# lightalchemist/nonlocal-image-edit

Hardware: AMD Instinct MI355X
Metric: megapixels/sec end-to-end enhance (4K img, m=200, K=50); device-resident input and output (host->host per SURVEY 8d: host_to_host.value) (higher is better)
Workload: dtype f64; 1 GPU; cfg4: 4096x4096 synthetic luminance, 20x10 samples (p=200), K=50, T=10, L=4 layers; device-resident: the luminance plane is in HBM when the timed region starts and the 4 layer planes are left in HBM (no PCIe inside `value`); parallelism=single GPU, formulation=phi_free_tables, storage=fp64 tables, histograms, reductions and MFMA; fp32 output planes

## Files before the change

include/nle.h:

```cpp
#ifndef NLE_H
#define NLE_H

#include <stddef.h>

#ifdef __cplusplus
extern "C" {
#endif

#define NLE_OK 0
#define NLE_ERR_INVALID 1
#define NLE_ERR_HIP 2
#define NLE_ERR_NUMERIC 3
#define NLE_ERR_COMM 4

#define NLE_EPS 1e-10

typedef struct nle_ctx nle_ctx;
typedef struct nle_filter nle_filter;

int nle_ctx_create(int device, void* stream, nle_ctx** out);
void nle_ctx_destroy(nle_ctx* ctx);
const char* nle_last_error(const nle_ctx* ctx);
int nle_ctx_synchronize(nle_ctx* ctx);
int nle_ctx_trim(nle_ctx* ctx);

int nle_dev_alloc(nle_ctx* ctx, size_t bytes, void** d_ptr);
void nle_dev_free(nle_ctx* ctx, void* d_ptr);
int nle_host_alloc(nle_ctx* ctx, size_t bytes, void** h_ptr);
void nle_host_free(nle_ctx* ctx, void* h_ptr);
int nle_dev_upload(nle_ctx* ctx, void* d_dst, const void* h_src, size_t bytes);
int nle_dev_download(nle_ctx* ctx, void* h_dst, const void* d_src, size_t bytes);

#define NLE_MODE_AUTO 0
#define NLE_MODE_MATERIALISED 1
#define NLE_MODE_PHI_FREE 2
#define NLE_MODE_PHI_FREE_EXP 3
#define NLE_MODE_MATERIALISED_F64 4
#define NLE_MODE_STREAMED_F64 5
#define NLE_MODE_EXACT_F64 6
#define NLE_EXACT_MAX_PIXELS 1048576
int nle_ctx_set_mode(nle_ctx* ctx, int mode);
#define NLE_PATCH_RADIUS_MAX 7
int nle_ctx_set_patch_radius(nle_ctx* ctx, int radius);
#define NLE_CHROMA_PATCH_RADIUS_MAX 3
int nle_ctx_set_chroma(nle_ctx* ctx, const float* d_a, const float* d_b, double hc);
int nle_filter_chroma(const nle_filter* f, double* hc);
#define NLE_SAMPLER_GRID 0
#define NLE_SAMPLER_FARTHEST 1
int nle_ctx_set_sampler(nle_ctx* ctx, int sampler);
int nle_sample_pixels(nle_ctx* ctx, const float* d_lum, int H, int W, int n_row_samples, int n_col_samples, double hx,
                      double hy, long long* h_idx, int* p);
int nle_ctx_set_nystrom_bf16x3(nle_ctx* ctx, int on);

int nle_ctx_set_slab_input(nle_ctx* ctx, int on);

int nle_ctx_set_topk_solver(nle_ctx* ctx, int solver);

#define NLE_RCCL_UNIQUE_ID_BYTES 128
int nle_rccl_unique_id(void* h_id, size_t size);
int nle_ctx_init_rccl(nle_ctx* ctx, int rank, int world, const void* h_id, size_t size);
int nle_ctx_set_rccl_comm(nle_ctx* ctx, int rank, int world, void* nccl_comm);
int nle_ctx_abort_rccl(nle_ctx* ctx);
typedef int (*nle_allreduce_fn)(void* user, void* d_buf, size_t count);
int nle_ctx_set_shard(nle_ctx* ctx, int rank, int world, nle_allreduce_fn allreduce,
                      void* user, double* d_comm, size_t comm_len);
size_t nle_comm_len(int n_samples);

int nle_sample_grid(int H, int W, int n_row_samples, int n_col_samples, int* row_step,
                    int* row_off, int* n_sel_rows, int* col_step, int* col_off,
                    int* n_sel_cols);
int nle_slab_rows(int H, int rank, int world, int* row0, int* row1);
int nle_eigen_decomposition(const double* h_M, int n, double eps, double* h_U, double* h_D,
                            int* r);
int nle_eigen_decomposition_top(const double* h_M, int n, double eps, int kmax, double* h_U, double* h_D, int* r);
int nle_eigen_decomposition_topk(const double* h_M, int n, double eps, int kmax, double* h_U, double* h_Dk, int* r);
int nle_eigen_decomposition_top_device(nle_ctx* ctx, const double* h_M, int n, double eps, int kmax, double* h_U, double* h_D,
                                       int* r);
int nle_sym_eigen_device(nle_ctx* ctx, const double* h_M, int n, double eps, int first, int count, double* h_U, double* h_D,
                         int* r);
int nle_cholesky_device(nle_ctx* ctx, const double* h_M, int n, double* h_L, double* h_Linv, double* inv_trace, int* ok);
int nle_topk_eigen_decomposition(const double* h_M, int n, int n_largest, double eps, double* h_U, double* h_D, int* r);
int nle_transform_eigenvalues(const double* h_eigvals, int K, const double* h_weights, int L,
                              double* h_fS);
int nle_layer_responses(const double* h_eigvals, int K, int L, double* h_resp);

int nle_compute_kernel(nle_ctx* ctx, const float* d_lum, int H, int W, int n_row_samples,
                       int n_col_samples, double hx, double hy, double* h_Ka, float* d_kab);
int nle_nystrom(nle_ctx* ctx, const float* d_lum, int H, int W, int n_row_samples,
                int n_col_samples, double hx, double hy, double* h_eigvals, int* r,
                float* d_phi);
int nle_ts_gemm(nle_ctx* ctx, const float* d_A, long long M, int lda, int kd,
                const double* h_B, int nc, float* d_C);
int nle_sinkhorn_scalings(nle_ctx* ctx, const float* d_phi, long long M, int ld, int r,
                          const double* h_eigvals, int max_iter, double* h_u_c,
                          double* h_u_r);
int nle_gram(nle_ctx* ctx, const float* d_phi, long long M, int ld, int r, const double* h_u,
             double* h_G);
int nle_row_scalings(nle_ctx* ctx, const float* d_phi, long long M, int ld, int r,
                     const double* h_u, double* d_out);

int nle_compute_kernel64(nle_ctx* ctx, const float* d_lum, int H, int W, int n_row_samples, int n_col_samples, double hx,
                         double hy, double* h_Ka, double* d_kab);
int nle_ts_gemm64(nle_ctx* ctx, const double* d_A, long long M, int lda, int kd, const double* h_B, int nc, double* d_C);
int nle_sinkhorn_scalings64(nle_ctx* ctx, const double* d_phi, long long M, int ld, int r, const double* h_eigvals,
                            int max_iter, double* h_u_c, double* h_u_r);
int nle_gram64(nle_ctx* ctx, const double* d_phi, long long M, int ld, int r, const double* h_u, double* h_G);
int nle_row_scalings64(nle_ctx* ctx, const double* d_phi, long long M, int ld, int r, const double* h_u, double* d_out);
int nle_affinity_product64(nle_ctx* ctx, const float* d_lum, int H, int W, double hx, double hy, const double* d_X, int ld,
                           int ncols, double* d_Y);

int nle_train(nle_ctx* ctx, const float* d_lum, int H, int W, int n_row_samples,
              int n_col_samples, double hx, double hy, int n_sinkhorn_iter,
              int n_eigen_vectors, nle_filter** out);
int nle_train_host(nle_ctx* ctx, const float* h_lum, int H, int W, int n_row_samples,
                   int n_col_samples, double hx, double hy, int n_sinkhorn_iter,
                   int n_eigen_vectors, nle_filter** out);
int nle_train_host_u8(nle_ctx* ctx, const unsigned char* h_lum8, int H, int W, int n_row_samples,
                      int n_col_samples, double hx, double hy, int n_sinkhorn_iter,
                      int n_eigen_vectors, nle_filter** out);
void nle_filter_destroy(nle_filter* f);
int nle_filter_info(const nle_filter* f, long long* n_local, int* K, int* r, int* p,
                    int* row0, int* row1);
int nle_filter_diag(const nle_filter* f, int* h_info);
int nle_filter_eigvals(const nle_filter* f, double* h_eigvals );
int nle_filter_sample_pixels(const nle_filter* f, long long* h_idx, int* p);
int nle_filter_eigvec_range(const nle_filter* f, int ncols, double* h_min, double* h_max);
int nle_filter_eigvecs(const nle_filter* f, const float** d_V, int* ld);
int nle_filter_copy_eigvecs(const nle_filter* f, float* d_out);
int nle_filter_timings(const nle_filter* f, double* h_ms);

int nle_apply(nle_filter* f, const float* d_x, int H, int W, const double* h_fS, float* d_y);
int nle_apply_layers(nle_filter* f, const float* d_x, int H, int W, int L, float* d_y);
int nle_apply_host(nle_filter* f, const float* h_x, int H, int W, const double* h_fS,
                   float* h_y);
int nle_apply_layers_host(nle_filter* f, const float* h_x, int H, int W, int L, float* h_y);
int nle_apply_u8(nle_filter* f, const float* d_x, int H, int W, const double* h_fS, unsigned char* d_out);
int nle_apply_rounded8(nle_filter* f, const float* d_x, int H, int W, const double* h_fS, float* d_y);
int nle_apply_u8_host(nle_filter* f, const float* h_x, int H, int W, const double* h_fS, unsigned char* h_out);

int nle_bgr2lab8(nle_ctx* ctx, const unsigned char* d_bgr, long long n, unsigned char* d_lab, float* d_L);
int nle_lab8_tables(unsigned short* h_gamma, unsigned short* h_cbrt, int* h_coeffs);
int nle_lab8_inverse_tables(unsigned short* h_yf, int* h_ab_to_xz, unsigned short* h_inv_gamma, int* h_coeffs);
int nle_lab2bgr8(nle_ctx* ctx, const unsigned char* d_lab, const float* d_L, long long n, unsigned char* d_bgr);
int nle_lab2bgr8_planes(nle_ctx* ctx, const unsigned char* d_lab, const float* d_L, const float* d_a, const float* d_b,
                        long long n, unsigned char* d_bgr);
int nle_lab8_channel(nle_ctx* ctx, const unsigned char* d_lab, long long n, int channel, float* d_out);

int nle_bilateral8(nle_ctx* ctx, const float* d_src, int H, int W, double sigma_color, double sigma_space, float* d_dst);
int nle_bilateral_tables(double sigma_color, double sigma_space, int* radius, float* h_space_w, float* h_colour_w);

int nle_ld(int n);

enum {
    NLE_K_AFFINITY = 0,
    NLE_K_NYSTROM = 1,
    NLE_K_SINKHORN_PASS = 2,
    NLE_K_REDUCE = 3,
    NLE_K_GRAM = 4,
    NLE_K_PROJECT = 5,
    NLE_K_APPLY_REDUCE = 6,
    NLE_K_APPLY_EXPAND = 7,
    NLE_K_SMALL = 8,
    NLE_K_SINK_TABLES = 9,
    NLE_K_GRAM_ROWS = 10,
    NLE_K_GRAM_GEMM = 11,
    NLE_KERNEL_COUNT = 12
};
const char* nle_kernel_name(int kid);
int nle_ctx_profile(nle_ctx* ctx, int enable);
int nle_ctx_kernel_stats(nle_ctx* ctx, int kid, long long* launches, double* total_ms);
int nle_bench_affinity(nle_ctx* ctx, const float* d_lum, int H, int W, int n_row_samples,
                       int n_col_samples, double hx, double hy, float* d_kab, int reps,
                       double* h_avg_ms);
int nle_bench_affinity64(nle_ctx* ctx, const float* d_lum, int H, int W, int n_row_samples, int n_col_samples, double hx,
                         double hy, long long rows, double* d_kab, int reps, double* h_avg_ms);
int nle_filter_level_tiles(const nle_filter* f, int* first_tile, int* n_tiles);
int nle_bench_sinkhorn_pass(nle_ctx* ctx, const float* d_phi, long long M, int ld, int r,
                            int reps, double* h_avg_ms);

#ifdef __cplusplus
}
#endif
#endif
```

nonlocal-image-edit_amd/__init__.py:

```python
from __future__ import annotations

import ctypes as C
import os

import numpy as np

_HERE = os.path.dirname(os.path.abspath(__file__))
LIB_PATH = os.path.join(_HERE, "lib", "libnle_hip.so")

from . import _abi
from ._abi import (ALLREDUCE_FN, NLE_ERR_COMM, NLE_ERR_HIP, NLE_ERR_INVALID, NLE_ERR_NUMERIC, NLE_OK)

EPS = 1e-10
KERNEL_COUNT = _abi.NLE_KERNEL_COUNT
_P = C.c_void_p
_SIGNATURES = _abi.SIGNATURES
EXPORTED_SYMBOLS = tuple(_SIGNATURES)
MODE_AUTO, MODE_MATERIALISED, MODE_PHI_FREE, MODE_PHI_FREE_EXP, MODE_MATERIALISED_F64, MODE_STREAMED_F64 = (
    _abi.NLE_MODE_AUTO, _abi.NLE_MODE_MATERIALISED, _abi.NLE_MODE_PHI_FREE, _abi.NLE_MODE_PHI_FREE_EXP,
    _abi.NLE_MODE_MATERIALISED_F64, _abi.NLE_MODE_STREAMED_F64)
MODE_EXACT_F64 = _abi.NLE_MODE_EXACT_F64
EXACT_MAX_PIXELS = _abi.NLE_EXACT_MAX_PIXELS
SAMPLER_GRID, SAMPLER_FARTHEST = _abi.NLE_SAMPLER_GRID, _abi.NLE_SAMPLER_FARTHEST

# ... 390 lines not shown
                                        float(hx), float(hy), _np_ptr(Ka),
                                        C.c_void_p(kab.data_ptr()) if want_kab else None), self._h)
        return np.ascontiguousarray(Ka), kab

    def nystrom(self, lum, n_row_samples, n_col_samples, hx, hy):
        torch = _torch()
        lum = self._lum(lum)
        H, W = lum.shape
        if n_row_samples > H or n_col_samples > W:
            raise NLEError(NLE_ERR_INVALID, "Number of samples per row and col must be <= that of image.")
        g = sample_grid(H, W, n_row_samples, n_col_samples)
        p = g["n_sel_rows"] * g["n_sel_cols"]
        n_local = self.local_pixels(H, W)
        buf = torch.empty(n_local * ld(p), dtype=torch.float32, device=lum.device)
        ev = np.zeros(p, dtype=np.float64)
        r = C.c_int()
        _check(lib().nle_nystrom(self._h, C.c_void_p(lum.data_ptr()), H, W, n_row_samples, n_col_samples, float(hx),
                                 float(hy), _np_ptr(ev), C.byref(r), C.c_void_p(buf.data_ptr())), self._h)
        rr = r.value
        return ev[:rr].copy(), buf[: n_local * ld(rr)].view(n_local, ld(rr)), rr

    def ts_gemm(self, A, kd, B):
        torch = _torch()
        self._sync_in()
        B = np.asfortranarray(np.asarray(B, dtype=np.float64))
        M, lda = A.shape
        nc = B.shape[1]
        Cc = torch.empty((M, ld(nc)), dtype=torch.float32, device=A.device)
        _check(lib().nle_ts_gemm(self._h, C.c_void_p(A.data_ptr()), M, lda, kd, _np_ptr(B), nc,
                                 C.c_void_p(Cc.data_ptr())), self._h)
        return Cc

    def sinkhorn_scalings(self, phi, r, eigvals, max_iter=10):
        ev = np.ascontiguousarray(eigvals, dtype=np.float64)
        uc, ur = np.zeros(r), np.zeros(r)
        self._sync_in()
        M, ldp = phi.shape
        _check(lib().nle_sinkhorn_scalings(self._h, C.c_void_p(phi.data_ptr()), M, ldp, r, _np_ptr(ev), max_iter,
                                           _np_ptr(uc), _np_ptr(ur)), self._h)
        return uc, ur

    def gram(self, phi, r, u):
        self._sync_in()
        u = np.ascontiguousarray(u, dtype=np.float64)
        G = np.zeros((r, r), dtype=np.float64, order="F")
        M, ldp = phi.shape
        _check(lib().nle_gram(self._h, C.c_void_p(phi.data_ptr()), M, ldp, r, _np_ptr(u), _np_ptr(G)), self._h)
        return np.ascontiguousarray(G)

    def row_scalings(self, phi, r, u):
        torch = _torch()
        self._sync_in()
        u = np.ascontiguousarray(u, dtype=np.float64)
        M, ldp = phi.shape
        out = torch.empty(M, dtype=torch.float64, device=phi.device)
        _check(lib().nle_row_scalings(self._h, C.c_void_p(phi.data_ptr()), M, ldp, r, _np_ptr(u),
                                      C.c_void_p(out.data_ptr())), self._h)
        return out

    def _mat64(self, X, width, what):
        torch = _torch()
        if X.dtype != torch.float64 or X.ndim != 2 or not X.is_cuda:
            raise NLEError(NLE_ERR_INVALID, f"{what}: need a float64 device tensor (M, ld)")
        M, ldx = X.shape
        if X.stride(1) != 1 or (M > 1 and X.stride(0) != ldx):
            raise NLEError(NLE_ERR_INVALID, f"{what}: rows must be contiguous with stride ld")
        if not 1 <= width <= ldx:
            raise NLEError(NLE_ERR_INVALID, f"{what}: need 1 <= logical width <= ld")
        self._sync_in()
        return M, ldx

    def ts_gemm64(self, A, kd, B):
        torch = _torch()
        M, lda = self._mat64(A, kd, "ts_gemm64")
        B = np.asfortranarray(np.asarray(B, dtype=np.float64))
        if B.ndim != 2 or B.shape[0] != kd:
            raise NLEError(NLE_ERR_INVALID, "ts_gemm64: B must be kd x nc")
        nc = B.shape[1]
        Cc = torch.empty((M, ld(nc)), dtype=torch.float64, device=A.device)
        _check(lib().nle_ts_gemm64(self._h, C.c_void_p(A.data_ptr()), M, lda, kd, _np_ptr(B), nc,
                                   C.c_void_p(Cc.data_ptr())), self._h)
        return Cc

    def sinkhorn_scalings64(self, phi, r, eigvals, max_iter=10):
        M, ldp = self._mat64(phi, r, "sinkhorn_scalings64")
        ev = np.ascontiguousarray(eigvals, dtype=np.float64)
        if ev.size < r:
            raise NLEError(NLE_ERR_INVALID, "sinkhorn_scalings64: need r eigenvalues")
        uc, ur = np.zeros(r), np.zeros(r)
        _check(lib().nle_sinkhorn_scalings64(self._h, C.c_void_p(phi.data_ptr()), M, ldp, r, _np_ptr(ev), max_iter,
                                             _np_ptr(uc), _np_ptr(ur)), self._h)
        return uc, ur

    def gram64(self, phi, r, u=None):
        M, ldp = self._mat64(phi, r, "gram64")
        if u is not None:
            u = np.ascontiguousarray(u, dtype=np.float64)
            if u.size < r:
                raise NLEError(NLE_ERR_INVALID, "gram64: need r entries of u")
        G = np.zeros((r, r), dtype=np.float64, order="F")
        _check(lib().nle_gram64(self._h, C.c_void_p(phi.data_ptr()), M, ldp, r, _np_ptr(u) if u is not None else None,
                                _np_ptr(G)), self._h)
        return np.ascontiguousarray(G)

    def row_scalings64(self, phi, r, u):
        torch = _torch()
        M, ldp = self._mat64(phi, r, "row_scalings64")
        u = np.ascontiguousarray(u, dtype=np.float64)
        if u.size < r:
            raise NLEError(NLE_ERR_INVALID, "row_scalings64: need r entries of u")
        out = torch.empty(M, dtype=torch.float64, device=phi.device)
        _check(lib().nle_row_scalings64(self._h, C.c_void_p(phi.data_ptr()), M, ldp, r, _np_ptr(u),
                                        C.c_void_p(out.data_ptr())), self._h)
        return out

    def bgr2lab8(self, bgr):
        torch = _torch()
        t = torch.as_tensor(bgr, dtype=torch.uint8, device=f"cuda:{self.device}").contiguous()
        self._sync_in()
        H, W = t.shape[:2]
        lab = torch.empty_like(t)
        L = torch.empty((H, W), dtype=torch.float32, device=t.device)
        _check(lib().nle_bgr2lab8(self._h, C.c_void_p(t.data_ptr()), H * W, C.c_void_p(lab.data_ptr()),
                                  C.c_void_p(L.data_ptr())), self._h)
        return lab, L

    def lab8_channel(self, lab, channel):
        torch = _torch()
        self._sync_in()
        H, W = lab.shape[:2]
        out = torch.empty((H, W), dtype=torch.float32, device=lab.device)
        _check(lib().nle_lab8_channel(self._h, C.c_void_p(lab.data_ptr()), H * W, int(channel),
                                      C.c_void_p(out.data_ptr())), self._h)
        return out

    def lab2bgr8(self, lab, L=None, a=None, b=None):
        torch = _torch()
        self._sync_in()
        H, W = lab.shape[:2]
        out = torch.empty_like(lab)
        ptr = lambda t: C.c_void_p(t.data_ptr()) if t is not None else None
        _check(lib().nle_lab2bgr8_planes(self._h, C.c_void_p(lab.data_ptr()), ptr(L), ptr(a), ptr(b), H * W,
                                         C.c_void_p(out.data_ptr())), self._h)
        return out

    def bilateral8(self, plane, sigma_color, sigma_space):
        torch = _torch()
        src = self._lum(plane)
        H, W = src.shape
        out = torch.empty_like(src)
        _check(lib().nle_bilateral8(self._h, C.c_void_p(src.data_ptr()), H, W, float(sigma_color), float(sigma_space),
                                    C.c_void_p(out.data_ptr())), self._h)
        return out

    def bench_affinity(self, lum, n_row_samples, n_col_samples, hx, hy, reps=10):
        torch = _torch()
        lum = self._lum(lum)
        H, W = lum.shape
        g = sample_grid(H, W, n_row_samples, n_col_samples)
        p = g["n_sel_rows"] * g["n_sel_cols"]
        kab = torch.empty((self.local_pixels(H, W), ld(p)), dtype=torch.float32, device=lum.device)
        ms = C.c_double()
        _check(lib().nle_bench_affinity(self._h, C.c_void_p(lum.data_ptr()), H, W, n_row_samples, n_col_samples,
                                        float(hx), float(hy), C.c_void_p(kab.data_ptr()), reps, C.byref(ms)), self._h)
        return ms.value, kab

# ... 226 lines not shown
```

nonlocal-image-edit_amd/_abi.py:

```python
import ctypes as C

_P = C.c_void_p

NLE_OK = 0
NLE_ERR_INVALID = 1
NLE_ERR_HIP = 2
NLE_ERR_NUMERIC = 3
NLE_ERR_COMM = 4
NLE_MODE_AUTO = 0
NLE_MODE_MATERIALISED = 1
NLE_MODE_PHI_FREE = 2
NLE_MODE_PHI_FREE_EXP = 3
NLE_MODE_MATERIALISED_F64 = 4
NLE_MODE_STREAMED_F64 = 5
NLE_MODE_EXACT_F64 = 6
NLE_EXACT_MAX_PIXELS = 1048576
NLE_PATCH_RADIUS_MAX = 7
NLE_CHROMA_PATCH_RADIUS_MAX = 3
NLE_SAMPLER_GRID = 0
NLE_SAMPLER_FARTHEST = 1
NLE_RCCL_UNIQUE_ID_BYTES = 128
NLE_K_AFFINITY = 0
NLE_K_NYSTROM = 1
NLE_K_SINKHORN_PASS = 2
NLE_K_REDUCE = 3
NLE_K_GRAM = 4
NLE_K_PROJECT = 5
NLE_K_APPLY_REDUCE = 6
NLE_K_APPLY_EXPAND = 7
NLE_K_SMALL = 8
NLE_K_SINK_TABLES = 9
NLE_K_GRAM_ROWS = 10
NLE_K_GRAM_GEMM = 11
NLE_KERNEL_COUNT = 12

ALLREDUCE_FN = C.CFUNCTYPE(C.c_int, _P, _P, C.c_size_t)

SIGNATURES = {
    "nle_ctx_create": (C.c_int, [C.c_int, _P, _P]),
    "nle_ctx_destroy": (None, [_P]),
    "nle_last_error": (C.c_char_p, [_P]),
    "nle_ctx_synchronize": (C.c_int, [_P]),
    "nle_ctx_trim": (C.c_int, [_P]),
    "nle_dev_alloc": (C.c_int, [_P, C.c_size_t, _P]),
    "nle_dev_free": (None, [_P, _P]),
    "nle_host_alloc": (C.c_int, [_P, C.c_size_t, _P]),
    "nle_host_free": (None, [_P, _P]),
    "nle_dev_upload": (C.c_int, [_P, _P, _P, C.c_size_t]),
    "nle_dev_download": (C.c_int, [_P, _P, _P, C.c_size_t]),
    "nle_ctx_set_mode": (C.c_int, [_P, C.c_int]),
    "nle_ctx_set_patch_radius": (C.c_int, [_P, C.c_int]),
    "nle_ctx_set_chroma": (C.c_int, [_P, _P, _P, C.c_double]),
    "nle_filter_chroma": (C.c_int, [_P, _P]),
    "nle_ctx_set_sampler": (C.c_int, [_P, C.c_int]),
    "nle_sample_pixels": (C.c_int, [_P, _P, C.c_int, C.c_int, C.c_int, C.c_int, C.c_double, C.c_double, _P, _P]),
    "nle_ctx_set_nystrom_bf16x3": (C.c_int, [_P, C.c_int]),
    "nle_ctx_set_slab_input": (C.c_int, [_P, C.c_int]),
    "nle_ctx_set_topk_solver": (C.c_int, [_P, C.c_int]),
    "nle_rccl_unique_id": (C.c_int, [_P, C.c_size_t]),
    "nle_ctx_init_rccl": (C.c_int, [_P, C.c_int, C.c_int, _P, C.c_size_t]),
    "nle_ctx_set_rccl_comm": (C.c_int, [_P, C.c_int, C.c_int, _P]),
    "nle_ctx_abort_rccl": (C.c_int, [_P]),
    "nle_ctx_set_shard": (C.c_int, [_P, C.c_int, C.c_int, ALLREDUCE_FN, _P, _P, C.c_size_t]),
    "nle_comm_len": (C.c_size_t, [C.c_int]),
    "nle_sample_grid": (C.c_int, [C.c_int, C.c_int, C.c_int, C.c_int, _P, _P, _P, _P, _P, _P]),
    "nle_slab_rows": (C.c_int, [C.c_int, C.c_int, C.c_int, _P, _P]),
    "nle_eigen_decomposition": (C.c_int, [_P, C.c_int, C.c_double, _P, _P, _P]),
    "nle_eigen_decomposition_top": (C.c_int, [_P, C.c_int, C.c_double, C.c_int, _P, _P, _P]),
    "nle_eigen_decomposition_topk": (C.c_int, [_P, C.c_int, C.c_double, C.c_int, _P, _P, _P]),
    "nle_eigen_decomposition_top_device": (C.c_int, [_P, _P, C.c_int, C.c_double, C.c_int, _P, _P, _P]),
    "nle_sym_eigen_device": (C.c_int, [_P, _P, C.c_int, C.c_double, C.c_int, C.c_int, _P, _P, _P]),
    "nle_cholesky_device": (C.c_int, [_P, _P, C.c_int, _P, _P, _P, _P]),
    "nle_topk_eigen_decomposition": (C.c_int, [_P, C.c_int, C.c_int, C.c_double, _P, _P, _P]),
    "nle_transform_eigenvalues": (C.c_int, [_P, C.c_int, _P, C.c_int, _P]),
    "nle_layer_responses": (C.c_int, [_P, C.c_int, C.c_int, _P]),
    "nle_compute_kernel": (C.c_int, [_P, _P, C.c_int, C.c_int, C.c_int, C.c_int, C.c_double, C.c_double, _P, _P]),
    "nle_nystrom": (C.c_int, [_P, _P, C.c_int, C.c_int, C.c_int, C.c_int, C.c_double, C.c_double, _P, _P, _P]),
    "nle_ts_gemm": (C.c_int, [_P, _P, C.c_longlong, C.c_int, C.c_int, _P, C.c_int, _P]),
    "nle_sinkhorn_scalings": (C.c_int, [_P, _P, C.c_longlong, C.c_int, C.c_int, _P, C.c_int, _P, _P]),
    "nle_gram": (C.c_int, [_P, _P, C.c_longlong, C.c_int, C.c_int, _P, _P]),
    "nle_row_scalings": (C.c_int, [_P, _P, C.c_longlong, C.c_int, C.c_int, _P, _P]),
    "nle_compute_kernel64": (C.c_int, [_P, _P, C.c_int, C.c_int, C.c_int, C.c_int, C.c_double, C.c_double, _P, _P]),
    "nle_ts_gemm64": (C.c_int, [_P, _P, C.c_longlong, C.c_int, C.c_int, _P, C.c_int, _P]),
    "nle_sinkhorn_scalings64": (C.c_int, [_P, _P, C.c_longlong, C.c_int, C.c_int, _P, C.c_int, _P, _P]),
    "nle_gram64": (C.c_int, [_P, _P, C.c_longlong, C.c_int, C.c_int, _P, _P]),
    "nle_row_scalings64": (C.c_int, [_P, _P, C.c_longlong, C.c_int, C.c_int, _P, _P]),
    "nle_affinity_product64": (C.c_int, [_P, _P, C.c_int, C.c_int, C.c_double, C.c_double, _P, C.c_int, C.c_int, _P]),
    "nle_train": (C.c_int, [_P, _P, C.c_int, C.c_int, C.c_int, C.c_int, C.c_double, C.c_double, C.c_int, C.c_int, _P]),
    "nle_train_host": (C.c_int, [_P, _P, C.c_int, C.c_int, C.c_int, C.c_int, C.c_double, C.c_double, C.c_int, C.c_int, _P]),
    "nle_train_host_u8": (C.c_int, [_P, _P, C.c_int, C.c_int, C.c_int, C.c_int, C.c_double, C.c_double, C.c_int, C.c_int, _P]),
    "nle_filter_destroy": (None, [_P]),
    "nle_filter_info": (C.c_int, [_P, _P, _P, _P, _P, _P, _P]),
    "nle_filter_diag": (C.c_int, [_P, _P]),
    "nle_filter_eigvals": (C.c_int, [_P, _P]),
    "nle_filter_sample_pixels": (C.c_int, [_P, _P, _P]),
    "nle_filter_eigvec_range": (C.c_int, [_P, C.c_int, _P, _P]),
    "nle_filter_eigvecs": (C.c_int, [_P, _P, _P]),
    "nle_filter_copy_eigvecs": (C.c_int, [_P, _P]),
    "nle_filter_timings": (C.c_int, [_P, _P]),
    "nle_apply": (C.c_int, [_P, _P, C.c_int, C.c_int, _P, _P]),
    "nle_apply_layers": (C.c_int, [_P, _P, C.c_int, C.c_int, C.c_int, _P]),
    "nle_apply_host": (C.c_int, [_P, _P, C.c_int, C.c_int, _P, _P]),
    "nle_apply_layers_host": (C.c_int, [_P, _P, C.c_int, C.c_int, C.c_int, _P]),
    "nle_apply_u8": (C.c_int, [_P, _P, C.c_int, C.c_int, _P, _P]),
    "nle_apply_rounded8": (C.c_int, [_P, _P, C.c_int, C.c_int, _P, _P]),
    "nle_apply_u8_host": (C.c_int, [_P, _P, C.c_int, C.c_int, _P, _P]),
    "nle_bgr2lab8": (C.c_int, [_P, _P, C.c_longlong, _P, _P]),
    "nle_lab8_tables": (C.c_int, [_P, _P, _P]),
    "nle_lab8_inverse_tables": (C.c_int, [_P, _P, _P, _P]),
    "nle_lab2bgr8": (C.c_int, [_P, _P, _P, C.c_longlong, _P]),
    "nle_lab2bgr8_planes": (C.c_int, [_P, _P, _P, _P, _P, C.c_longlong, _P]),
    "nle_lab8_channel": (C.c_int, [_P, _P, C.c_longlong, C.c_int, _P]),
    "nle_bilateral8": (C.c_int, [_P, _P, C.c_int, C.c_int, C.c_double, C.c_double, _P]),
    "nle_bilateral_tables": (C.c_int, [C.c_double, C.c_double, _P, _P, _P]),
    "nle_ld": (C.c_int, [C.c_int]),
    "nle_kernel_name": (C.c_char_p, [C.c_int]),
    "nle_ctx_profile": (C.c_int, [_P, C.c_int]),
    "nle_ctx_kernel_stats": (C.c_int, [_P, C.c_int, _P, _P]),
    "nle_bench_affinity": (C.c_int, [_P, _P, C.c_int, C.c_int, C.c_int, C.c_int, C.c_double, C.c_double, _P, C.c_int, _P]),
    "nle_bench_affinity64": (C.c_int, [_P, _P, C.c_int, C.c_int, C.c_int, C.c_int, C.c_double, C.c_double, C.c_longlong, _P, C.c_int, _P]),
    "nle_filter_level_tiles": (C.c_int, [_P, _P, _P]),
    "nle_bench_sinkhorn_pass": (C.c_int, [_P, _P, C.c_longlong, C.c_int, C.c_int, C.c_int, _P]),
}
```

nonlocal-image-edit_amd/csrc/abi_ctx.hip:

```cpp
#include <mutex>

#include "lab8_fixed.h"
#include "pipeline_internal.h"

using nlek::GridSpec;
using namespace nlep;

extern "C" {

int nle_ld(int n) { return ld4(n); }

size_t nle_comm_len(int n_samples) {
    const int ld = ld4(n_samples);
    return std::max(std::max((size_t)nlek::gram_num_tiles(ld) * 1024, (size_t)nlek::gram64_num_tiles(n_samples) * 256),
                    (size_t)n_samples * n_samples) +
           8 * (size_t)nlek::sink_pass_ld(n_samples);
}

int nle_ctx_create(int device, void* stream, nle_ctx** out) {
    if (!out) return NLE_ERR_INVALID;
    *out = nullptr;
    return guard(nullptr, [&] {
        int ndev = 0;
        HIP_OK(hipGetDeviceCount(&ndev));
// ... 386 lines not shown
}

int nle_ctx_set_shard(nle_ctx* ctx, int rank, int world, nle_allreduce_fn allreduce, void* user,
                      double* d_comm, size_t comm_len) {
    if (!ctx) return NLE_ERR_INVALID;
    return guard(ctx, [&] {
        if (world < 1 || rank < 0 || rank >= world) throw Fail{NLE_ERR_INVALID, "bad rank/world"};
        if (world > 1 && (!allreduce || !d_comm || comm_len == 0))
            throw Fail{NLE_ERR_INVALID, "world > 1 needs an all-reduce callback and a comm buffer"};
        ctx->rank = rank;
        ctx->world = world;
        ctx->allreduce = allreduce;
        ctx->ar_user = user;
        ctx->d_comm = d_comm;
        ctx->comm_len = comm_len;
    });
}

int nle_sample_grid(int H, int W, int n_row_samples, int n_col_samples, int* row_step, int* row_off,
                    int* n_sel_rows, int* col_step, int* col_off, int* n_sel_cols) {
    GridSpec gs;
    if (!make_grid(H, W, n_row_samples, n_col_samples, &gs)) return NLE_ERR_INVALID;
    if (row_step) *row_step = gs.rowStep;
    if (row_off) *row_off = gs.rowOff;
    if (n_sel_rows) *n_sel_rows = gs.nSelRows;
    if (col_step) *col_step = gs.colStep;
    if (col_off) *col_off = gs.colOff;
    if (n_sel_cols) *n_sel_cols = gs.nSelCols;
    return NLE_OK;
}

int nle_slab_rows(int H, int rank, int world, int* row0, int* row1) {
    if (H <= 0 || world < 1 || rank < 0 || rank >= world || !row0 || !row1) return NLE_ERR_INVALID;
    slab(H, rank, world, row0, row1);
    return NLE_OK;
}

int nle_eigen_decomposition(const double* h_M, int n, double eps, double* h_U, double* h_D, int* r) {
    if (!h_M || n <= 0 || !h_U || !h_D || !r) return NLE_ERR_INVALID;
    return nleh::eigen_decomposition(h_M, n, eps, h_U, h_D, r) ? NLE_OK : NLE_ERR_NUMERIC;
}

int nle_transform_eigenvalues(const double* h_eigvals, int K, const double* h_weights, int L, double* h_fS) {
    if (!h_eigvals || !h_weights || !h_fS || K < 0 || L < 1) return NLE_ERR_INVALID;
    for (int i = 0; i < K; ++i) {
        double v = h_weights[0];
        for (int k = 1; k < L; ++k) v += (h_weights[k] - h_weights[k - 1]) * std::pow(h_eigvals[i], (double)k);
        h_fS[i] = v;
    }
    return NLE_OK;
}

static const char* const kKernelNames[NLE_KERNEL_COUNT] = {
    "affinity", "nystrom_extend", "sinkhorn_pass", "reduce_partials", "gram",
    "project",  "apply_reduce",   "apply_expand",  "small",           "sink_tables", "gram_rows",
    "gram_gemm"};

const char* nle_kernel_name(int kid) { return (kid >= 0 && kid < NLE_KERNEL_COUNT) ? kKernelNames[kid] : ""; }

int nle_ctx_profile(nle_ctx* ctx, int enable) {
    if (!ctx) return NLE_ERR_INVALID;
    return guard(ctx, [&] {
        HIP_OK(hipStreamSynchronize(ctx->stream));
        prof_flush(ctx);
        ctx->profiling = enable != 0;
        ctx->profile_all = enable >= 2;
        for (int k = 0; k < NLE_KERNEL_COUNT; ++k) {
            ctx->prof_launches[k] = 0;
            ctx->prof_ms[k] = 0.0;
        }
    });
}

int nle_ctx_kernel_stats(nle_ctx* ctx, int kid, long long* launches, double* total_ms) {
    if (!ctx || kid < 0 || kid >= NLE_KERNEL_COUNT) return NLE_ERR_INVALID;
    return guard(ctx, [&] {
        HIP_OK(hipStreamSynchronize(ctx->stream));
        prof_flush(ctx);
        if (launches) *launches = ctx->prof_launches[kid];
        if (total_ms) *total_ms = ctx->prof_ms[kid];
    });
}

}
```

nonlocal-image-edit_amd/csrc/fused.hip:

```cpp
#include "kernels.h"

#include <algorithm>
#include <cstdlib>

namespace nlek {

typedef float f32x16 __attribute__((ext_vector_type(16)));

__device__ __forceinline__ double recip_or_zero_d(double s, double eps) {
    return (fabs(s) >= eps) ? 1.0 / s : 0.0;
}

template <int MASK>
__device__ __forceinline__ void fold_level(float& a, float& b, int lane) {
    if constexpr (MASK == 32) {
        auto r = __builtin_amdgcn_permlane32_swap(__float_as_uint(a), __float_as_uint(b), false, false);
        a = __uint_as_float(r[0]) + __uint_as_float(r[1]);
    } else if constexpr (MASK == 16) {
        auto r = __builtin_amdgcn_permlane16_swap(__float_as_uint(a), __float_as_uint(b), false, false);
        a = __uint_as_float(r[0]) + __uint_as_float(r[1]);
    } else {
        const bool hi = (lane & MASK) != 0;
        const float keep = hi ? b : a, give = hi ? a : b;
        a = keep + __shfl_xor(give, MASK);
// ... 711 lines not shown
    }
}

hipError_t check_levels(hipStream_t s, const float* d_lum, long long n, int* d_flag) {
    hipError_t e = hipMemsetAsync(d_flag, 0, 2 * sizeof(int), s);
    if (e != hipSuccess) return e;
    long long g = (n + 255) / 256;
    if (g > 1024) g = 1024;
    hipLaunchKernelGGL(k_check_levels, dim3((unsigned)g), dim3(256), 0, s, d_lum, n, d_flag);
    return hipGetLastError();
}

__global__ void k_hist_tables(GridSpec gs, const Sample4* __restrict__ samples, int p, double inv_hx2,
                              double inv_hy2, int row0, int nrows_local, double* __restrict__ er,
                              double* __restrict__ ecT, double* __restrict__ Ep) {
    const long long n_er = (long long)nrows_local * gs.nSelRows, n_ec = (long long)gs.nSelCols * gs.W,
                    n_ep = (long long)kLevels * p;
    for (long long i = (long long)blockIdx.x * blockDim.x + threadIdx.x; i < n_er + n_ec + n_ep;
         i += (long long)gridDim.x * blockDim.x) {
        if (i < n_er) {
            const int r = row0 + (int)(i / gs.nSelRows), a = (int)(i % gs.nSelRows);
            const double d = (double)(r - (gs.rowOff + a * gs.rowStep));
            er[i] = exp(-(d * d) * inv_hx2);
        } else if (i < n_er + n_ec) {
            const long long j = i - n_er;
            const int b = (int)(j / gs.W), c = (int)(j % gs.W);
            const double d = (double)(c - (gs.colOff + b * gs.colStep));
            ecT[j] = exp(-(d * d) * inv_hx2);
        } else {
            const long long j = i - n_er - n_ec;
            const int x = (int)(j / p), sidx = (int)(j % p);
            const double d = (double)x - (double)samples[sidx].z;
            Ep[j] = exp(-(d * d) * inv_hy2);
        }
    }
}

hipError_t hist_tables(hipStream_t s, GridSpec gs, const Sample4* d_samples, int p, double hx, double hy, int row0,
                       int nrows_local, double* d_er, double* d_ecT, double* d_Ep) {
    hipLaunchKernelGGL(k_hist_tables, dim3(256), dim3(256), 0, s, gs, d_samples, p, 1.0 / (hx * hx), 1.0 / (hy * hy),
                       row0, nrows_local, d_er, d_ecT, d_Ep);
    return hipGetLastError();
}

__global__ __launch_bounds__(256) void k_hist_g(GridSpec gs, int p, int nrows, int tiles_per_wave, int lev_t0, int lev_nt,
                                                const double* __restrict__ er, const double* __restrict__ Ep,
                                                const double* __restrict__ w, double* __restrict__ g) {
    extern __shared__ __attribute__((aligned(16))) unsigned char smem_raw[];
    double* sEr = reinterpret_cast<double*>(smem_raw);
    const int nC = gs.nSelCols, nR = gs.nSelRows, n = kLevels * nC;
    const int tid = threadIdx.x, lane = tid & 63, wave = tid >> 6, l15 = lane & 15, kq = lane >> 4;
    const int t0 = blockIdx.y * tiles_per_wave, ntiles = (nrows + 15) >> 4;
    const int rbase = t0 * 16, rcount = min(nrows - rbase, tiles_per_wave * 16);
    for (int i = tid; i < rcount * nR; i += 256) sEr[i] = er[(size_t)rbase * nR + i];
    const int q = blockIdx.x * 4 + wave;
    const bool col_ok = q < nC * lev_nt;
    const int b = col_ok ? q / lev_nt : 0, x = (lev_t0 + (col_ok ? q % lev_nt : 0)) * 16 + l15;
    const int col = b * kLevels + x;
    double bop[8];
#pragma unroll
    for (int ks = 0; ks < 8; ++ks) {
        const int a = ks * 4 + kq;
        bop[ks] = (col_ok && a < nR) ? w[a * nC + b] * Ep[(size_t)x * p + a * nC + b] : 0.0;
    }
    __syncthreads();
    if (!col_ok) return;
    const int ksteps = (nR + 3) >> 2;
    for (int t = t0; t < min(ntiles, t0 + tiles_per_wave); ++t) {
        const int rl = (t - t0) * 16 + l15;
        double aop[8];
#pragma unroll
        for (int ks = 0; ks < 8; ++ks) {
            const int a = ks * 4 + kq;
            aop[ks] = (ks < ksteps && rl < rcount && a < nR) ? sEr[rl * nR + a] : 0.0;
        }
        f64x4 acc = f64x4{0.0, 0.0, 0.0, 0.0};
#pragma unroll
        for (int ks = 0; ks < 8; ++ks)
            if (ks < ksteps) acc = __builtin_amdgcn_mfma_f64_16x16x4f64(aop[ks], bop[ks], acc, 0, 0, 0);
        if (col_ok) {
#pragma unroll
            for (int e = 0; e < 4; ++e) {
                const int ro = t * 16 + kq + 4 * e;
                if (ro < nrows) g[(size_t)ro * n + col] = acc[e];
            }
        }
    }
}

static hipError_t launch_hist_g(hipStream_t s, GridSpec gs, int p, int nrows_local, const double* d_er, const double* d_Ep,
                                const double* d_w, double* d_g, int lev_t0 = 0, int lev_nt = kLevels / 16) {
    const int ntiles = (nrows_local + 15) / 16;
    const int gx = (gs.nSelCols * lev_nt + 3) / 4;
    const int cap = gs.nSelRows > 24 ? 8 : 16;
    const int chunks = std::max(1, std::min(ntiles, std::max((640 + gx - 1) / gx, (ntiles + cap - 1) / cap)));
    const int tpw = (ntiles + chunks - 1) / chunks;
    const size_t shm = (size_t)tpw * 16 * gs.nSelRows * sizeof(double);
    if (shm > 48 * 1024) {
        hipError_t ea = hipFuncSetAttribute(reinterpret_cast<const void*>(k_hist_g), hipFuncAttributeMaxDynamicSharedMemorySize,
                                            (int)shm);
        if (ea != hipSuccess) return ea;
    }
    hipLaunchKernelGGL(k_hist_g, dim3((unsigned)gx, (unsigned)((ntiles + tpw - 1) / tpw)), dim3(256), shm, s, gs, p,
                       nrows_local, tpw, lev_t0, lev_nt, d_er, d_Ep, d_w, d_g);
    return hipGetLastError();
}

constexpr int kPixThreads = 512;
template <int NC>
__global__ __launch_bounds__(kPixThreads) void k_hist_pix(int mode, const float* __restrict__ lum, GridSpec gs, int row0,
                                                  const double* __restrict__ ecT, const double* __restrict__ g,
                                                  double eps, double* __restrict__ ybuf, double* __restrict__ hout,
                                                  const double* __restrict__ cvec, const float* __restrict__ xvec) {
    extern __shared__ __attribute__((aligned(16))) unsigned char smem_raw[];
    constexpr int n = kLevels * NC;
    constexpr int NS = NC | 1;
    const int W = gs.W;
    double* sg = reinterpret_cast<double*>(smem_raw);
    double* sh = sg + kLevels * NS;
    const int tid = threadIdx.x, lrow = blockIdx.x, r = row0 + lrow;
    const double* grow = g + (size_t)lrow * n;
    for (int i = tid; i < n; i += kPixThreads) {
        const int bb = i / kLevels, xx = i & (kLevels - 1);
        sh[xx * NS + bb] = 0.0;
        sg[xx * NS + bb] = (mode == ROWPASS_RECIP) ? grow[i] : 0.0;
    }
    __syncthreads();
    const int dr = r - gs.rowOff;
    const bool sample_row = dr >= 0 && (dr % gs.rowStep) == 0 && (dr / gs.rowStep) < gs.nSelRows;
    for (int c0 = 0; c0 < W; c0 += kPixThreads) {
        const bool inside = c0 + tid < W;
        const int c = inside ? c0 + tid : W - 1;
        const int x = (int)lum[(size_t)r * W + c];
        bool smp = !inside;
        if (sample_row) {
            const int dc = c - gs.colOff;
            smp = smp || (dc >= 0 && (dc % gs.colStep) == 0 && (dc / gs.colStep) < NC);
        }
        double e[NC];
#pragma unroll
        for (int b = 0; b < NC; ++b) e[b] = ecT[(size_t)b * W + c];
        double y = 1.0;
        if (mode == ROWPASS_XVEC) {
            y = cvec[(size_t)lrow * W + c] * (double)xvec[(size_t)r * W + c];
        } else if (mode == ROWPASS_RECIP) {
            double gv[NC];
#pragma unroll
            for (int b = 0; b < NC; ++b) gv[b] = sg[x * NS + b];
            double s0 = 0.0, s1 = 0.0;
#pragma unroll
            for (int b = 0; b < NC; ++b) {
                if (b & 1) s1 += e[b] * gv[b];
                else s0 += e[b] * gv[b];
            }
            y = recip_or_zero_d(s0 + s1, eps);
        }
        if (smp) y = 0.0;
        if (ybuf != nullptr && inside) ybuf[(size_t)lrow * W + c] = y;
        const bool own = wave_group_levels(y != 0.0, x, [&](int lx, bool mine) {
#pragma unroll
            for (int b = 0; b < NC; ++b) {
                const double t = wave_sum63(mine ? e[b] * y : 0.0);
                if ((tid & 63) == 63) atomicAdd(&sh[lx * NS + b], t);
            }
        });
        if (own) {
#pragma unroll
// ... 102 lines not shown
__global__ void k_scatter_samples(int p, int L, const long long* __restrict__ loc, const double* __restrict__ YA,
                                  float* __restrict__ Y, long long ystride, int round8) {
    const int o = blockIdx.x * blockDim.x + threadIdx.x;
    if (o >= L * p) return;
    const int l = o / p, a = o - l * p;
    double v = YA[o];
    if (round8) v = rint(fmin(255.0, fmax(0.0, v)));
    if (loc[a] >= 0) Y[(size_t)l * ystride + loc[a]] = (float)v;
}

__global__ __launch_bounds__(256) void k_hist_hh(int nC, int nR, int nrows, int slab_rows, int lev_t0, int lev_nt,
                                                 const double* __restrict__ er, const double* __restrict__ h,
                                                 const double* __restrict__ Ep, int p, int ldp, double* __restrict__ zpart) {
    extern __shared__ __attribute__((aligned(16))) unsigned char smem_raw[];
    double* sEr = reinterpret_cast<double*>(smem_raw);
    const int n = kLevels * nC;
    const int tid = threadIdx.x, lane = tid & 63, wave = tid >> 6, l15 = lane & 15, kq = lane >> 4;
    const int r0 = blockIdx.y * slab_rows, rcount = min(nrows - r0, slab_rows);
    for (int i = tid; i < rcount * nR; i += 256) sEr[i] = er[(size_t)r0 * nR + i];
    const int q = blockIdx.x * 4 + wave;
    const bool col_ok = q < nC * lev_nt;
    const int b = col_ok ? q / lev_nt : 0, xt = lev_t0 + (col_ok ? q % lev_nt : 0), x = xt * 16 + l15;
    const int col = b * kLevels + x;
    const bool two = nR > 16;
    f64x4 acc0 = f64x4{0.0, 0.0, 0.0, 0.0}, acc1 = acc0;
    __syncthreads();
    if (!col_ok) return;
    for (int k0 = 0; k0 < slab_rows; k0 += 64) {
        double bop[16];
#pragma unroll
        for (int ks = 0; ks < 16; ++ks) {
            const int rl = k0 + ks * 4 + kq;
            bop[ks] = (col_ok && rl < rcount) ? h[(size_t)(r0 + rl) * n + col] : 0.0;
        }
#pragma unroll
        for (int ks = 0; ks < 16; ++ks) {
            const int rl = k0 + ks * 4 + kq;
            const bool rok = rl < rcount;
            const double a0 = (rok && l15 < nR) ? sEr[rl * nR + l15] : 0.0;
            acc0 = __builtin_amdgcn_mfma_f64_16x16x4f64(a0, bop[ks], acc0, 0, 0, 0);
            if (two) {
                const double a1 = (rok && 16 + l15 < nR) ? sEr[rl * nR + 16 + l15] : 0.0;
                acc1 = __builtin_amdgcn_mfma_f64_16x16x4f64(a1, bop[ks], acc1, 0, 0, 0);
            }
        }
    }
    double v[8];
#pragma unroll
    for (int e = 0; e < 4; ++e) {
        const int a0 = kq + 4 * e, a1 = 16 + kq + 4 * e;
        v[e] = (col_ok && a0 < nR) ? acc0[e] * Ep[(size_t)x * p + a0 * nC + b] : 0.0;
        v[4 + e] = (two && col_ok && a1 < nR) ? acc1[e] * Ep[(size_t)x * p + a1 * nC + b] : 0.0;
    }
#pragma unroll
    for (int off = 1; off < 16; off <<= 1)
#pragma unroll
        for (int e = 0; e < 8; ++e) v[e] += __shfl_xor(v[e], off);
    if (l15 == 0 && col_ok) {
        double* out = zpart + ((size_t)blockIdx.y * lev_nt + (xt - lev_t0)) * ldp;
#pragma unroll
        for (int e = 0; e < 4; ++e) {
            const int a0 = kq + 4 * e, a1 = 16 + kq + 4 * e;
            if (a0 < nR) out[a0 * nC + b] = v[e];
            if (two && a1 < nR) out[a1 * nC + b] = v[4 + e];
        }
    }
}

__global__ __launch_bounds__(256) void k_z_reduce(const double* __restrict__ zpart, int nparts, int p, int ldp,
                                                  double* __restrict__ z) {
    __shared__ double sm[32][8];
    const int c = threadIdx.x & 7, g = threadIdx.x >> 3, col = blockIdx.x * 8 + c;
    double s = 0.0;
    if (col < p)
        for (int r = g; r < nparts; r += 32) s += zpart[(size_t)r * ldp + col];
    sm[g][c] = s;
    __syncthreads();
    if (g == 0 && col < ldp) {
        double t = 0.0;
#pragma unroll
        for (int k = 0; k < 32; ++k) t += sm[k][c];
        z[col] = t;
    }
}

int hist_tiled_max_rows_samples() { return 32; }
static int hist_slab_rows(GridSpec gs, int nrows_local) {
    const int ncoltiles = kLevels * gs.nSelCols / 16;
    const int want = std::max(1, (4096 + ncoltiles - 1) / ncoltiles);
    int rows = (nrows_local + want - 1) / want;
    rows = std::max(64, ((rows + 31) / 32) * 32);
    const int lds_rows = ((8192 / std::max(gs.nSelRows, 1)) / 32) * 32;
    return std::min(rows, std::max(64, lds_rows));
}
size_t hist_tiled_workspace_elems(GridSpec gs, int nrows_local) {
    const size_t n = (size_t)kLevels * gs.nSelCols;
    const int sr = hist_slab_rows(gs, nrows_local);
    const int nslabs = (nrows_local + sr - 1) / sr;
    const size_t ldp = ((size_t)gs.nSelRows * gs.nSelCols + 63) & ~(size_t)63;
    return 2 * (size_t)nrows_local * n + (size_t)nslabs * std::max(n * gs.nSelRows, (size_t)(kLevels / 16) * ldp);
}

hipError_t sink_hist_tiled(hipStream_t s, int mode, const float* d_lum, GridSpec gs, int p, int ldp, int row0,
                           int nrows_local, const double* d_er, const double* d_ecT, const double* d_Ep,
                           const double* d_w, double eps, double* d_ybuf, double* d_ws, double* d_z,
                           LaunchObserver* obs, const double* d_cvec, const float* d_xvec, const SortedRows* sorted) {
    const int nC = gs.nSelCols, nR = gs.nSelRows;
    if (nC > 36 || nR > 32) return hipErrorInvalidValue;
    struct Scope {
        LaunchObserver* o;
        Scope(LaunchObserver* ob, int sub) : o(ob) { if (o) o->begin(sub); }
        ~Scope() { if (o) o->end(); }
    };
    const size_t n = (size_t)kLevels * nC;
    const int slab_rows = hist_slab_rows(gs, nrows_local), nslabs = (nrows_local + slab_rows - 1) / slab_rows;
    double* d_g = d_ws;
    double* d_h = d_g + (size_t)nrows_local * n;
    double* d_HH = d_h + (size_t)nrows_local * n;
    const int lev_t0 = sorted ? sorted->lev_t0 : 0, lev_nt = sorted ? sorted->lev_nt : kLevels / 16;
    if (mode == ROWPASS_RECIP) {
        Scope sc(obs, SUB_HIST_G);
        hipError_t eg = launch_hist_g(s, gs, p, nrows_local, d_er, d_Ep, d_w, d_g, lev_t0, lev_nt);
        if (eg != hipSuccess) return eg;
    }
    if (sorted != nullptr) {
        Scope sc(obs, SUB_HIST_PIX);
        hipError_t ep = sorted_pass(s, mode, gs, row0, nrows_local, sorted->scol, sorted->desc, sorted->first, sorted->E, d_g,
                                    eps, d_ybuf, d_h, d_cvec, d_xvec, sorted->rec, sorted->kappa, lev_t0, lev_nt, sorted->mom);
        if (ep != hipSuccess) return ep;
    } else {
        Scope sc(obs, SUB_HIST_PIX);
#define NLE_HP(NCV)                                                                                                 \
    case NCV:                                                                                                       \
        hipLaunchKernelGGL((k_hist_pix<NCV>), dim3((unsigned)nrows_local), dim3(kPixThreads),                      \
                           (size_t)2 * kLevels * ((NCV) | 1) * sizeof(double), s, mode,                            \
                           d_lum, gs, row0, d_ecT, d_g, eps, d_ybuf, d_h, d_cvec, d_xvec);                          \
        break;
        if (nC > 11) {
            hipError_t ea = hipSuccess;
            switch (nC) {
#define NLE_HPA(NCV) case NCV: ea = hipFuncSetAttribute(reinterpret_cast<const void*>(k_hist_pix<NCV>), hipFuncAttributeMaxDynamicSharedMemorySize, (int)(2 * kLevels * ((NCV) | 1) * sizeof(double))); break;
                NLE_HPA(12) NLE_HPA(13) NLE_HPA(14) NLE_HPA(15) NLE_HPA(16) NLE_HPA(17) NLE_HPA(18) NLE_HPA(19) NLE_HPA(20)
                NLE_HPA(21) NLE_HPA(22) NLE_HPA(23) NLE_HPA(24) NLE_HPA(25) NLE_HPA(26) NLE_HPA(27) NLE_HPA(28) NLE_HPA(29)
                NLE_HPA(30) NLE_HPA(31) NLE_HPA(32) NLE_HPA(33) NLE_HPA(34) NLE_HPA(35) NLE_HPA(36)
#undef NLE_HPA
                default: break;
            }
            if (ea != hipSuccess) return ea;
        }
        switch (nC) {
            NLE_HP(1) NLE_HP(2) NLE_HP(3) NLE_HP(4) NLE_HP(5) NLE_HP(6) NLE_HP(7) NLE_HP(8) NLE_HP(9) NLE_HP(10) NLE_HP(11)
            NLE_HP(12) NLE_HP(13) NLE_HP(14) NLE_HP(15) NLE_HP(16) NLE_HP(17) NLE_HP(18) NLE_HP(19) NLE_HP(20)
            NLE_HP(21) NLE_HP(22) NLE_HP(23) NLE_HP(24) NLE_HP(25) NLE_HP(26) NLE_HP(27) NLE_HP(28) NLE_HP(29)
            NLE_HP(30) NLE_HP(31) NLE_HP(32) NLE_HP(33) NLE_HP(34) NLE_HP(35) NLE_HP(36)
            default: return hipErrorInvalidValue;
        }
#undef NLE_HP
    }
    Scope sc(obs, SUB_HIST_HH);
    {
        const size_t shm_hh = (size_t)slab_rows * nR * sizeof(double);
        if (shm_hh > 48 * 1024) {
            hipError_t ea = hipFuncSetAttribute(reinterpret_cast<const void*>(k_hist_hh),
                                                hipFuncAttributeMaxDynamicSharedMemorySize, (int)shm_hh);
            if (ea != hipSuccess) return ea;
        }
        hipLaunchKernelGGL(k_hist_hh, dim3((unsigned)((nC * lev_nt + 3) / 4), (unsigned)nslabs), dim3(256), shm_hh, s, nC, nR,
                           nrows_local, slab_rows, lev_t0, lev_nt, d_er, d_h, d_Ep, p, ldp, d_HH);
    }
    hipLaunchKernelGGL(k_z_reduce, dim3((unsigned)((ldp + 7) / 8)), dim3(256), 0, s, d_HH, nslabs * lev_nt, p, ldp, d_z);
    return hipGetLastError();
}

int apply_layers_per_launch(GridSpec gs) {
    const size_t table = (size_t)kLevels * (gs.nSelCols | 1) * sizeof(double);
    return (int)std::max<size_t>(1, std::min<size_t>(kDotLayers, (size_t)(144 * 1024) / table));
}

bool use_sorted_expand(GridSpec gs, const SortedRows* sorted) {
    return sorted != nullptr && gs.nSelCols <= sorted_expand_max_cols() && gs.W <= sorted_expand_max_width();
}

hipError_t apply_hist_layers(hipStream_t s, const float* d_lum, GridSpec gs, int p, int row0, int nrows_local,
                             const double* d_er, const double* d_ecT, const double* d_Ep, const double* d_wl, int ldw,
                             int nl, const double* d_c, double* d_ws, float* d_out, long long ostride,
                             LaunchObserver* obs, const SortedRows* sorted, bool round8) {
    const int nC = gs.nSelCols, nR = gs.nSelRows;
    if (nC > 36 || nR > 32 || nrows_local <= 0) return nrows_local <= 0 ? hipSuccess : hipErrorInvalidValue;
    const bool use_sorted = use_sorted_expand(gs, sorted);
    if (nl < 1 || nl > (use_sorted ? sorted_expand_layers(gs) : apply_layers_per_launch(gs))) return hipErrorInvalidValue;
    const size_t n = (size_t)kLevels * nC, gstride = (size_t)nrows_local * n;
    if (obs) obs->begin(SUB_HIST_G);
    for (int l = 0; l < nl; ++l) {
        hipError_t eg = launch_hist_g(s, gs, p, nrows_local, d_er, d_Ep, d_wl + (size_t)l * ldw, d_ws + (size_t)l * gstride,
                                      use_sorted ? sorted->lev_t0 : 0, use_sorted ? sorted->lev_nt : kLevels / 16);
        if (eg != hipSuccess) return eg;
    }
    if (obs) obs->end(), obs->begin(SUB_HIST_PIX);
    if (use_sorted) {
        hipError_t ex = sorted_expand(s, gs, nrows_local, sorted->scol, sorted->desc, sorted->E, d_ws, gstride, nl, d_c, d_out,
                                      ostride, sorted->rec, sorted->kappa, round8);
        if (obs) obs->end();
        return ex;
    }
#define NLE_HD(NCV)                                                                                                  \
    case NCV: {                                                                                                      \
        const size_t shm_d = (size_t)nl * kLevels * ((NCV) | 1) * sizeof(double);                                    \
        if (shm_d > 48 * 1024) {                                                                                     \
            hipError_t ea = hipFuncSetAttribute(reinterpret_cast<const void*>(k_hist_dot<NCV>),                      \
                                                hipFuncAttributeMaxDynamicSharedMemorySize, (int)shm_d);             \
            if (ea != hipSuccess) return ea;                                                                         \
        }                                                                                                            \
        hipLaunchKernelGGL((k_hist_dot<NCV>), dim3((unsigned)nrows_local), dim3(kDotThreads), shm_d, s, d_lum, gs,   \
                           row0, d_ecT, d_ws, gstride, nl, d_c, d_out, ostride, round8 ? 1 : 0);                     \
    } break;
    switch (nC) {
        NLE_HD(1) NLE_HD(2) NLE_HD(3) NLE_HD(4) NLE_HD(5) NLE_HD(6) NLE_HD(7) NLE_HD(8) NLE_HD(9) NLE_HD(10) NLE_HD(11)
        NLE_HD(12) NLE_HD(13) NLE_HD(14) NLE_HD(15) NLE_HD(16) NLE_HD(17) NLE_HD(18) NLE_HD(19) NLE_HD(20)
        NLE_HD(21) NLE_HD(22) NLE_HD(23) NLE_HD(24) NLE_HD(25) NLE_HD(26) NLE_HD(27) NLE_HD(28) NLE_HD(29)
        NLE_HD(30) NLE_HD(31) NLE_HD(32) NLE_HD(33) NLE_HD(34) NLE_HD(35) NLE_HD(36)
        default: return hipErrorInvalidValue;
    }
#undef NLE_HD
    if (obs) obs->end();
    return hipGetLastError();
}

hipError_t apply_small(hipStream_t s, int p, int K, int ldk, int L, int ldw, const double* d_m, const double* d_D,
                       const double* d_Vrows, const double* d_xA, const double* d_resp, double* d_t, double* d_Wp,
                       double* d_YA) {
    const size_t shm = (size_t)(2 * p + K + 256) * sizeof(double);
    hipLaunchKernelGGL(k_apply_small, dim3((unsigned)L), dim3(256), shm, s, p, K, ldk, L, ldw, d_m, d_D, d_Vrows, d_xA,
                       d_resp, d_t, d_Wp, d_YA);
    return hipGetLastError();
}

hipError_t scatter_samples(hipStream_t s, int p, int L, const long long* d_loc, const double* d_YA, float* d_Y,
                           long long ystride, bool round8) {
    hipLaunchKernelGGL(k_scatter_samples, dim3((unsigned)((L * p + 255) / 256)), dim3(256), 0, s, p, L, d_loc, d_YA, d_Y,
                       ystride, round8 ? 1 : 0);
    return hipGetLastError();
}

int ghist_max_cols() { return 36; }

__device__ __forceinline__ int tri_index(int i, int j, int n) {
    return i * n - (i * (i - 1)) / 2 + (j - i);
}

constexpr int kGhistRowsThreads = 512;
__global__ __launch_bounds__(kGhistRowsThreads) void k_ghist_rows(const float* __restrict__ lum, GridSpec gs, int row0,
                                                    const double* __restrict__ ecT,
                                                    const double* __restrict__ cvec, double* __restrict__ Aout) {
    extern __shared__ __attribute__((aligned(16))) unsigned char smem_raw[];
// ... 360 lines not shown
```

nonlocal-image-edit_amd/csrc/generic64.hip:

```cpp
#include "kernels.h"

#include <algorithm>

namespace nlek {

typedef double f64x4 __attribute__((ext_vector_type(4)));

namespace {
__device__ __forceinline__ double recip0_g(double s, double eps) {
    return (fabs(s) >= eps) ? 1.0 / s : 0.0;
}
}

constexpr int kAff64Pix = 64;

template <bool CHROMA>
__global__ __launch_bounds__(256) void k_affinity64(const float* __restrict__ lum, GridSpec gs,
                                                    const Sample4* __restrict__ samples, int p, int ld, double sw,
                                                    double pw, long long pix0, long long M, double* __restrict__ kab,
                                                    int skip_samples, const unsigned* __restrict__ smask,
                                                    const float* __restrict__ pa, const float* __restrict__ pb,
                                                    const float2* __restrict__ sab, double cw) {
    extern __shared__ __attribute__((aligned(16))) unsigned char smem_raw64[];
    int2* srow_col = reinterpret_cast<int2*>(smem_raw64);
// ... 87 lines not shown
                       a.samples, a.p, a.ld, a.sw, a.pw, pix0, M, d_kab, skip_samples ? 1 : 0, a.smask, a.a, a.b, a.sab, a.cw);
    return hipGetLastError();
}
}

hipError_t patch_affinity_rows64(hipStream_t s, const Affinity64Args& a, long long pix0, long long M, double* d_kab,
                                 bool skip_samples);
hipError_t affinity_rows64(hipStream_t s, const Affinity64Args& a, long long pix0, long long M, double* d_kab,
                           bool skip_samples) {
    if (M <= 0) return hipSuccess;
    if (a.R > 0) return patch_affinity_rows64(s, a, pix0, M, d_kab, skip_samples);
    return a.a ? launch_affinity64_chroma(s, a, pix0, M, d_kab, skip_samples)
               : launch_affinity64(s, a, pix0, M, d_kab, skip_samples);
}

__global__ void k_add64(double* __restrict__ y, const double* __restrict__ x, size_t n) {
    for (size_t i = blockIdx.x * (size_t)blockDim.x + threadIdx.x; i < n; i += (size_t)gridDim.x * blockDim.x) y[i] += x[i];
}
hipError_t add64(hipStream_t s, double* d_y, const double* d_x, size_t n) {
    if (n == 0) return hipSuccess;
    hipLaunchKernelGGL(k_add64, dim3((unsigned)std::min<size_t>((n + 255) / 256, 2048)), dim3(256), 0, s, d_y, d_x, n);
    return hipGetLastError();
}

__global__ __launch_bounds__(256) void k_row_scalings64(const double* __restrict__ X, long long M, int ld, int r,
                                                        const double* __restrict__ u, double eps, double* __restrict__ out) {
    const int lane = threadIdx.x & 63;
    const long long wv = (long long)blockIdx.x * 4 + (threadIdx.x >> 6), nw = (long long)gridDim.x * 4;
    for (long long i = wv; i < M; i += nw) {
        double s = 0.0;
        for (int j = lane; j < r; j += 64) s += X[(size_t)i * ld + j] * u[j];
#pragma unroll
        for (int off = 32; off > 0; off >>= 1) s += __shfl_xor(s, off);
        if (lane == 0) out[i] = recip0_g(s, eps);
    }
}

hipError_t row_scalings64(hipStream_t s, const double* d_X, long long M, int ld, int r, const double* d_u, double eps,
                          double* d_out) {
    if (M <= 0) return hipSuccess;
    const long long nb = std::min<long long>((M + 3) / 4, 8192);
    hipLaunchKernelGGL(k_row_scalings64, dim3((unsigned)nb), dim3(256), 0, s, d_X, M, ld, r, d_u, eps, d_out);
    return hipGetLastError();
}

__global__ __launch_bounds__(256) void k_tsgemm64(const double* __restrict__ A, long long M, int lda, int kd,
                                                  const double* __restrict__ B, int nc, const double* __restrict__ rs,
                                                  double* __restrict__ C, int ldc) {
    const int lane = threadIdx.x & 63, wave = threadIdx.x >> 6, l15 = lane & 15, kq = lane >> 4;
    const int ctiles = (nc + 15) / 16;
    const long long rtiles = (M + 15) / 16, ntiles = rtiles * ctiles;
    for (long long t = (long long)blockIdx.x * 4 + wave; t < ntiles; t += (long long)gridDim.x * 4) {
        const long long rt = t / ctiles;
        const int ct = (int)(t - rt * ctiles);
        const long long arow = rt * 16 + l15;
        const int bcol = ct * 16 + l15;
        const bool aok = arow < M, bok = bcol < nc;
        f64x4 acc = f64x4{0.0, 0.0, 0.0, 0.0};
        for (int k0 = 0; k0 < kd; k0 += 4) {
            const int k = k0 + kq;
            const double a = (aok && k < kd) ? A[(size_t)arow * lda + k] : 0.0;
            const double b = (bok && k < kd) ? B[(size_t)bcol * kd + k] : 0.0;
            acc = __builtin_amdgcn_mfma_f64_16x16x4f64(a, b, acc, 0, 0, 0);
        }
        if (bok) {
#pragma unroll
            for (int e = 0; e < 4; ++e) {
                const long long ro = rt * 16 + kq + 4 * e;
                if (ro < M) C[(size_t)ro * ldc + bcol] = (rs ? rs[ro] : 1.0) * acc[e];
            }
        }
    }
}

hipError_t ts_gemm64(hipStream_t s, const double* d_A, long long M, int lda, int kd, const double* d_B, int nc,
                     const double* d_rs, double* d_C, int ldc) {
    if (M <= 0 || nc <= 0) return hipSuccess;
    const long long ntiles = ((M + 15) / 16) * ((nc + 15) / 16);
    const long long nb = std::min<long long>((ntiles + 3) / 4, 65535);
    hipLaunchKernelGGL(k_tsgemm64, dim3((unsigned)nb), dim3(256), 0, s, d_A, M, lda, kd, d_B, nc, d_rs, d_C, ldc);
    return hipGetLastError();
}

__global__ __launch_bounds__(256) void k_gemm64s(int m, int n, int kk, const double* __restrict__ A, long long rsA,
                                                 long long csA, const double* __restrict__ B, long long rsB, long long csB,
                                                 double* __restrict__ C, long long rsC, long long csC,
                                                 const double* __restrict__ dl, const double* __restrict__ dk,
                                                 const double* __restrict__ dr, const double* __restrict__ add,
                                                 long long rsD, long long csD) {
    const int lane = threadIdx.x & 63, wave = threadIdx.x >> 6, l15 = lane & 15, kq = lane >> 4;
    const int ct = (n + 15) / 16, rt = (m + 15) / 16;
    const int t = blockIdx.x * 4 + wave;
    if (t >= rt * ct) return;
    const int ti = t / ct, tj = t - ti * ct;
    const int ai = ti * 16 + l15, bj = tj * 16 + l15;
    const bool aok = ai < m, bok = bj < n;
    const double* ap = A + (long long)ai * rsA;
    const double* bp = B + (long long)bj * csB;
    f64x4 acc = f64x4{0.0, 0.0, 0.0, 0.0};
    for (int k0 = 0; k0 < kk; k0 += 16) {
        double a[4], b[4];
#pragma unroll
        for (int u = 0; u < 4; ++u) {
            const int k = k0 + 4 * u + kq;
            const bool kok = k < kk;
            a[u] = (aok && kok) ? ap[(long long)k * csA] * (dk ? dk[k] : 1.0) : 0.0;
            b[u] = (bok && kok) ? bp[(long long)k * rsB] : 0.0;
        }
#pragma unroll
        for (int u = 0; u < 4; ++u) acc = __builtin_amdgcn_mfma_f64_16x16x4f64(a[u], b[u], acc, 0, 0, 0);
    }
    if (bok) {
        const double sr = dr ? dr[bj] : 1.0;
#pragma unroll
        for (int e = 0; e < 4; ++e) {
            const int ro = ti * 16 + kq + 4 * e;
            if (ro < m) {
                double v = (dl ? dl[ro] : 1.0) * acc[e] * sr;
                if (add) v += add[(long long)ro * rsD + (long long)bj * csD];
                C[(long long)ro * rsC + (long long)bj * csC] = v;
            }
        }
    }
}

hipError_t gemm64s(hipStream_t s, int m, int n, int kk, const double* A, long long rsA, long long csA, const double* B,
                   long long rsB, long long csB, double* C, long long rsC, long long csC, const double* dl, const double* dk,
                   const double* dr, const double* add, long long rsD, long long csD) {
    if (m <= 0 || n <= 0) return hipSuccess;
    const long long ntiles = (long long)((m + 15) / 16) * ((n + 15) / 16);
    hipLaunchKernelGGL(k_gemm64s, dim3((unsigned)((ntiles + 3) / 4)), dim3(256), 0, s, m, n, kk, A, rsA, csA, B, rsB, csB, C, rsC,
                       csC, dl, dk, dr, add, rsD, csD);
    return hipGetLastError();
}

constexpr int kRp64Cols = 32;

template <int NCL>
__global__ __launch_bounds__(256) void k_rowpass64(int mode, const double* __restrict__ X, long long M, int ld, int w, int lw,
                                                   const double* __restrict__ t_in, const double* __restrict__ lam,
                                                   const float* __restrict__ xvec, double eps, double* __restrict__ partial) {
    extern __shared__ __attribute__((aligned(16))) unsigned char smem_raw[];
    double* sred = reinterpret_cast<double*>(smem_raw);
    const int lane = threadIdx.x & 63, wave = threadIdx.x >> 6;
    double u[NCL], acc[NCL];
#pragma unroll
    for (int k = 0; k < NCL; ++k) {
        const int j = lane + 64 * k;
        u[k] = (mode == ROWPASS_RECIP && j < w) ? lam[j] * t_in[j] : 0.0;
        acc[k] = 0.0;
    }
    const long long wv = (long long)blockIdx.x * 4 + wave, nw = (long long)gridDim.x * 4;
    for (long long i = wv; i < M; i += nw) {
        double v[NCL];
        double s = 0.0;
#pragma unroll
        for (int k = 0; k < NCL; ++k) {
            const int j = lane + 64 * k;
            v[k] = (j < w) ? X[(size_t)i * ld + j] : 0.0;
            s += v[k] * u[k];
        }
        double y = 1.0;
        if (mode == ROWPASS_RECIP) {
#pragma unroll
            for (int off = 32; off > 0; off >>= 1) s += __shfl_xor(s, off);
            y = recip0_g(s, eps);
        } else if (mode == ROWPASS_XVEC) {
            y = (double)xvec[i];
        }
#pragma unroll
        for (int k = 0; k < NCL; ++k) acc[k] += v[k] * y;
    }
#pragma unroll
    for (int k = 0; k < NCL; ++k) {
        const int j = lane + 64 * k;
        if (j < lw) sred[wave * lw + j] = acc[k];
    }
    __syncthreads();
    for (int j = threadIdx.x; j < lw; j += 256)
        partial[(size_t)blockIdx.x * lw + j] = (sred[j] + sred[lw + j]) + (sred[2 * lw + j] + sred[3 * lw + j]);
}

hipError_t rowpass64(hipStream_t s, int mode, const double* d_X, long long M, int ld, int w, const double* d_t_in,
                     const double* d_lam, const float* d_xvec, double eps, double* d_partial, int* nblocks) {
    if (w < 1 || w > ld || w > 64 * kRp64Cols) return hipErrorInvalidValue;
    const int lw = (w + 3) & ~3;
    long long nb = (M + 3) / 4;
    nb = std::max<long long>(1, std::min<long long>(nb, kRowpassMaxBlocks));
    *nblocks = (int)nb;
    const size_t shm = (size_t)4 * lw * sizeof(double);
#define NLE_RP64(NCLV)                                                                                                  \
    {                                                                                                                   \
        if (shm > 48 * 1024) {                                                                                          \
            hipError_t ea = hipFuncSetAttribute(reinterpret_cast<const void*>(k_rowpass64<NCLV>),                       \
// ... 63 lines not shown
    return rows;
}
size_t gram64d_partial_elems(long long M, int r) {
    const long long rows = gram64d_chunk_rows(M);
    const long long nchunks = std::max<long long>(1, (M + rows - 1) / rows);
    return (size_t)nchunks * r * r;
}

hipError_t gram64d(hipStream_t s, const double* d_X, long long M, int ld, int r, const double* d_cs, double* d_partial,
                   double* d_G) {
    const long long rows = gram64d_chunk_rows(M);
    const int nchunks = (int)std::max<long long>(1, (M + rows - 1) / rows);
    const int nt = (r + 15) / 16, npairs = nt * (nt + 1) / 2;
    hipError_t e = hipMemsetAsync(d_partial, 0, (size_t)nchunks * r * r * sizeof(double), s);
    if (e != hipSuccess) return e;
    if (M > 0)
        hipLaunchKernelGGL(k_gram64d, dim3((unsigned)((npairs + 3) / 4), (unsigned)nchunks), dim3(256), 0, s, d_X, M, ld, r, d_cs,
                           rows, d_partial);
    hipLaunchKernelGGL(k_gram64d_reduce, dim3((unsigned)(((long long)r * r + 255) / 256)), dim3(256), 0, s, d_partial, nchunks, r,
                       d_G);
    return hipGetLastError();
}

__global__ __launch_bounds__(256) void k_apply_expand64(const double* __restrict__ V, long long M, int ld, int K,
                                                        const double* __restrict__ g, int L, float* __restrict__ Y,
                                                        long long ystride) {
    extern __shared__ __attribute__((aligned(16))) unsigned char smem_raw[];
    double* sg = reinterpret_cast<double*>(smem_raw);
    for (int j = threadIdx.x; j < L * K; j += 256) sg[j] = g[(size_t)(j / K) * ld + (j % K)];
    __syncthreads();
    for (long long i = (long long)blockIdx.x * 256 + threadIdx.x; i < M; i += (long long)gridDim.x * 256) {
        const double* v = V + (size_t)i * ld;
        for (int l = 0; l < L; ++l) {
            double s0 = 0.0, s1 = 0.0;
            int k = 0;
            for (; k + 1 < K; k += 2) {
                s0 += v[k] * sg[l * K + k];
                s1 += v[k + 1] * sg[l * K + k + 1];
            }
            if (k < K) s0 += v[k] * sg[l * K + k];
            Y[(size_t)l * ystride + i] = (float)(s0 + s1);
        }
    }
}

hipError_t apply_expand64(hipStream_t s, const double* d_V, long long M, int ld, int K, const double* d_g, int L, float* d_Y,
                          long long ystride) {
    if (M <= 0 || L <= 0) return hipSuccess;
    const size_t per_layer = (size_t)K * sizeof(double);
    if (per_layer > kApplyLdsBytes) return hipErrorInvalidValue;
    const int lmax = per_layer ? (int)std::min<size_t>(kApplyLdsBytes / per_layer, (size_t)L) : L;
    const int ngroups = (L + lmax - 1) / lmax, lg = (L + ngroups - 1) / ngroups;
    const long long nb = std::min<long long>((M + 255) / 256, 4096);
    for (int l0 = 0; l0 < L; l0 += lg) {
        const int ln = std::min(lg, L - l0);
        const size_t shm = (size_t)ln * per_layer;
        if (shm > 48 * 1024) {
            hipError_t ea = hipFuncSetAttribute(reinterpret_cast<const void*>(k_apply_expand64),
                                                hipFuncAttributeMaxDynamicSharedMemorySize, (int)shm);
            if (ea != hipSuccess) return ea;
        }
        hipLaunchKernelGGL(k_apply_expand64, dim3((unsigned)nb), dim3(256), shm, s, d_V, M, ld, K, d_g + (size_t)l0 * ld, ln,
                           d_Y + (size_t)l0 * ystride, ystride);
    }
    return hipGetLastError();
}

__global__ void k_scatter_rows64(const double* __restrict__ src, const long long* __restrict__ idx, int n, int ld,
                                 double* __restrict__ X, long long M) {
    const long long f = (long long)blockIdx.x * blockDim.x + threadIdx.x;
    if (f >= (long long)n * ld) return;
    const int k = (int)(f / ld), j = (int)(f % ld);
    const long long row = idx[k];
    if (row >= 0 && row < M) X[(size_t)row * ld + j] = src[f];
}

hipError_t scatter_rows64(hipStream_t s, const double* d_src, const long long* d_idx, int n, int ld, double* d_X, long long M) {
    if (n <= 0) return hipSuccess;
    hipLaunchKernelGGL(k_scatter_rows64, dim3((unsigned)(((long long)n * ld + 255) / 256)), dim3(256), 0, s, d_src, d_idx, n, ld,
                       d_X, M);
    return hipGetLastError();
}

__global__ void k_scale_rows64(double* __restrict__ X, int m, int n, const double* __restrict__ dl) {
    const long long f = (long long)blockIdx.x * blockDim.x + threadIdx.x;
    if (f < (long long)m * n) X[f] *= dl[f % m];
}
hipError_t scale_rows64(hipStream_t s, double* d_X, int m, int n, const double* d_dl) {
    if (m <= 0 || n <= 0) return hipSuccess;
    hipLaunchKernelGGL(k_scale_rows64, dim3((unsigned)(((long long)m * n + 255) / 256)), dim3(256), 0, s, d_X, m, n, d_dl);
    return hipGetLastError();
}

__global__ void k_to_f32(const double* __restrict__ X, long long n, float* __restrict__ out) {
    for (long long i = (long long)blockIdx.x * blockDim.x + threadIdx.x; i < n; i += (long long)gridDim.x * blockDim.x)
        out[i] = (float)X[i];
}
hipError_t to_f32(hipStream_t s, const double* d_X, long long n, float* d_out) {
    if (n <= 0) return hipSuccess;
    hipLaunchKernelGGL(k_to_f32, dim3((unsigned)std::min<long long>((n + 255) / 256, 8192)), dim3(256), 0, s, d_X, n, d_out);
    return hipGetLastError();
}

}
```

nonlocal-image-edit_amd/csrc/kernels.h:

```cpp
#pragma once
#include <hip/hip_runtime.h>

#include <vector>

namespace nlek {

struct GridSpec {
    int H, W;
    int rowStep, rowOff, nSelRows;
    int colStep, colOff, nSelCols;
    __host__ __device__ int p() const { return nSelRows * nSelCols; }
};

typedef float4 Sample4;

#if defined(__HIPCC__)
__device__ __forceinline__ float affinity_value(float pr, float pc, float px, Sample4 s, float nsw, float npw) {
    const float dr = pr - s.x, dc = pc - s.y, dv = px - s.z;
    return __builtin_amdgcn_exp2f(nsw * (dr * dr + dc * dc) + npw * (dv * dv));
}
__device__ __forceinline__ bool is_sample_pixel(const GridSpec& gs, int row, int col) {
    const int dr = row - gs.rowOff, dc = col - gs.colOff;
    if (dr < 0 || dc < 0) return false;
    const int qr = dr / gs.rowStep, qc = dc / gs.colStep;
// ... 45 lines not shown
hipError_t scale_vec(hipStream_t s, const double* d_lam, const double* d_t, int n, double* d_u);
hipError_t row_scalings(hipStream_t s, const float* d_X, long long M, int ld, const double* d_u,
                        double eps, double* d_out);

int gram_num_tiles(int ld);
int gram_chunk_rows(long long M);
size_t gram_partial_elems(long long M, int ld);
hipError_t gram(hipStream_t s, const float* d_X, long long M, int ld, const double* d_u,
                double eps, double* d_partial, double* d_tiles);
hipError_t gram_reduce(hipStream_t s, const double* d_partial, int nchunks, int ntiles, double* d_tiles);

int sink_pass_ld(int p);
int sink_pass_rows(long long M);
int sink_pass_max_p();
hipError_t sink_pass(hipStream_t s, int mode, const float* d_lum, GridSpec gs, const Sample4* d_samples,
                     int p, const double* d_w, float nsw, float npw, long long pix0, long long M, double eps,
                     double* d_ybuf, double* d_partial);
hipError_t sink_update(hipStream_t s, int mode, int p, int r, bool chol, const double* d_X1, const double* d_X2,
                       const double* d_lam, const double* d_z, int zrows, int zld, const double* d_sA_cur, double eps,
                       double* d_v, double* d_u, double* d_sA_next, double* d_w_next);
constexpr int kG64TilesPerWave = 23;
int gram64_ld(int p);
int gram64_num_tiles(int p);
size_t gram64_partial_elems(long long M, int p);
hipError_t gram64(hipStream_t s, const float* d_lum, GridSpec gs, const Sample4* d_samples, int p, float nsw,
                  float npw, long long pix0, long long M, const double* d_c, double* d_partial, double* d_tiles);
int project64_ld(int K);
hipError_t project64(hipStream_t s, const float* d_lum, GridSpec gs, const Sample4* d_samples, int p, float nsw,
                     float npw, long long pix0, long long M, const double* d_D, int K, const double* d_c, float* d_V,
                     int ldv);

hipError_t check_levels(hipStream_t s, const float* d_lum, long long n, int* d_flag);
hipError_t hist_tables(hipStream_t s, GridSpec gs, const Sample4* d_samples, int p, double hx, double hy, int row0,
                       int nrows_local, double* d_er, double* d_ecT, double* d_Ep);

struct Affinity64Args {
    const float* lum = nullptr;
    GridSpec gs{};
    const Sample4* samples = nullptr;
    int p = 0, ld = 0;
    double sw = 0.0, pw = 0.0;
    int R = 0;
    const signed char *spatch = nullptr, *cpatch = nullptr;
    const int *snorm = nullptr, *cnorm = nullptr;
    const float *a = nullptr, *b = nullptr;
    double cw = 0.0;
    const float2* sab = nullptr;
    const unsigned* smask = nullptr;
};
constexpr size_t kDynLdsDefault = 64 * 1024;
constexpr size_t kPatchChromaLdsMax = 128 * 1024;
size_t affinity64_chroma_lds_bytes(int ld);
size_t patch_affinity64_chroma_lds_bytes(int ld);
int patch_kpad(int R);
int patch_ckpad(int R);
size_t patch_spatch_bytes(int p, int R);
size_t patch_cpatch_bytes(int p, int R);
hipError_t affinity_rows64(hipStream_t s, const Affinity64Args& a, long long pix0, long long M, double* d_kab,
                           bool skip_samples);
hipError_t patch_gather(hipStream_t s, const float* d_lum, int H, int W, int R, const long long* d_pix, int n, int* d_out);
int farthest_max_blocks();
hipError_t farthest_samples(hipStream_t s, const float* d_lum, int H, int W, int p, double sw, double pw, double* d_m,
                            double* d_pv, int* d_pi, int* d_list);
hipError_t gather_pix(hipStream_t s, const float* d_lum, const long long* d_pix, int n, float* d_out);
hipError_t sample_mask(hipStream_t s, const long long* d_pix, int n, long long N, unsigned* d_mask);
hipError_t add64(hipStream_t s, double* d_y, const double* d_x, size_t n);
hipError_t row_scalings64(hipStream_t s, const double* d_X, long long M, int ld, int r, const double* d_u, double eps,
                          double* d_out);
hipError_t ts_gemm64(hipStream_t s, const double* d_A, long long M, int lda, int kd, const double* d_B, int nc,
                     const double* d_rs, double* d_C, int ldc);
hipError_t gemm64s(hipStream_t s, int m, int n, int kk, const double* A, long long rsA, long long csA, const double* B,
                   long long rsB, long long csB, double* C, long long rsC, long long csC, const double* dl = nullptr,
                   const double* dk = nullptr, const double* dr = nullptr, const double* add = nullptr, long long rsD = 0,
                   long long csD = 0);
hipError_t rowpass64(hipStream_t s, int mode, const double* d_X, long long M, int ld, int w, const double* d_t_in,
                     const double* d_lam, const float* d_xvec, double eps, double* d_partial, int* nblocks);
size_t gram64d_partial_elems(long long M, int r);
hipError_t gram64d(hipStream_t s, const double* d_X, long long M, int ld, int r, const double* d_cs, double* d_partial,
                   double* d_G);
hipError_t apply_expand64(hipStream_t s, const double* d_V, long long M, int ld, int K, const double* d_g, int L, float* d_Y,
                          long long ystride);
hipError_t scatter_rows64(hipStream_t s, const double* d_src, const long long* d_idx, int n, int ld, double* d_X, long long M);
hipError_t to_f32(hipStream_t s, const double* d_X, long long n, float* d_out);
hipError_t scale_rows64(hipStream_t s, double* d_X, int m, int n, const double* d_dl);

int tridiag_max_n();
hipError_t tridiag(hipStream_t s, int n, const double* d_Q, const double* d_diag_add, double* d_V, double* d_d, double* d_e,
                   double* d_hs);

int sytrd_max_n();
int sytrd_groups(int n);
size_t sytrd_pub_elems(int n);
hipError_t sytrd_dist(hipStream_t s, int n, int G, const double* d_A, const double* d_diag_add, double* d_pub, double* d_d,
                      double* d_e, int* d_status);
hipError_t tridiag_bisect(hipStream_t s, int n, const double* d_d, const double* d_e, double* d_D);
hipError_t sytrd_back(hipStream_t s, int n, const double* d_pub, int K, double* d_Z, int ldz);
size_t potrf_tmp_elems(int n);
hipError_t potrf_inverse(hipStream_t s, int n, const double* d_A, double* d_L, double* d_Linv, double* d_tmp, double* d_scal,
                         int* d_status);
hipError_t transpose64(hipStream_t s, int n, const double* d_src, double* d_dst, int lds = 0, int ldd = 0);
hipError_t symm_lower64(hipStream_t s, int n, const double* d_src, double* d_dst);
hipError_t fill64(hipStream_t s, double* d_p, size_t n, double v);
hipError_t scale_rc64(hipStream_t s, int n, const double* d_src, int lds, const double* d_dl, const double* d_dr, double* d_dst);

constexpr int kSortedThreads = 512;
struct SortedRows {
    const unsigned short* scol;
    const uint2* desc;
    const unsigned short* first;
    const double* E;
    bool rec;
    double kappa;
    const double* E2 = nullptr;
    double hx = 0.0;
    int lev_t0 = 0, lev_nt = 16;
    bool mom = false;
};
bool sorted_gsum_ok(GridSpec gs, double hx);
hipError_t sorted_gram_sums(hipStream_t s, GridSpec gs, int nrows_local, const unsigned short* d_scol, const uint2* d_desc,
                            const unsigned short* d_first, const double* d_E2, const double* d_cvec, double* d_Aout, double hx);
bool sorted_recurrence(GridSpec gs, double hx, double* kappa);
int sorted_max_width();
size_t sorted_scol_elems(int W, int nrows_local);
int sorted_gram_max_cols();
int sorted_expand_max_cols();
int sorted_expand_max_width();
int sorted_expand_layers(GridSpec gs);
hipError_t sorted_expand(hipStream_t s, GridSpec gs, int nrows_local, const unsigned short* d_scol, const uint2* d_desc,
                         const double* d_E, const double* d_g, size_t gstride, int nl, const double* d_cvec, float* d_out,
                         long long ostride, bool rec = false, double kappa = 0.0, bool round8 = false);
hipError_t dist_table(hipStream_t s, int W, double hx, double* d_E);
hipError_t sort_rows(hipStream_t s, const float* d_lum, GridSpec gs, int row0, int nrows_local, unsigned short* d_scol,
                     uint2* d_desc, unsigned short* d_first);
hipError_t sorted_pass(hipStream_t s, int mode, GridSpec gs, int row0, int nrows_local, const unsigned short* d_scol,
                       const uint2* d_desc, const unsigned short* d_first, const double* d_E, const double* d_g, double eps,
                       double* d_ybuf, double* d_h, const double* d_cvec, const float* d_xvec, bool rec, double kappa,
                       int lev_t0 = 0, int lev_nt = 16,
                       bool mom = false);
bool sorted_moments_ok(GridSpec gs, double hx);
hipError_t sorted_gram_rows(hipStream_t s, GridSpec gs, int nrows_local, const unsigned short* d_scol, const uint2* d_desc,
                            const unsigned short* d_first, const double* d_E, const double* d_cvec, double* d_Aout, bool rec,
                            double kappa);

size_t hist_tiled_workspace_elems(GridSpec gs, int nrows_local);
hipError_t sink_hist_tiled(hipStream_t s, int mode, const float* d_lum, GridSpec gs, int p, int ldp, int row0,
                           int nrows_local, const double* d_er, const double* d_ecT, const double* d_Ep,
                           const double* d_w, double eps, double* d_ybuf, double* d_ws, double* d_z,
                           LaunchObserver* obs = nullptr, const double* d_cvec = nullptr,
                           const float* d_xvec = nullptr,
                           const SortedRows* sorted = nullptr);
int apply_layers_per_launch(GridSpec gs);
bool use_sorted_expand(GridSpec gs, const SortedRows* sorted);
hipError_t apply_hist_layers(hipStream_t s, const float* d_lum, GridSpec gs, int p, int row0, int nrows_local,
                             const double* d_er, const double* d_ecT, const double* d_Ep, const double* d_wl, int ldw,
                             int nl, const double* d_c, double* d_ws, float* d_out, long long ostride,
                             LaunchObserver* obs, const SortedRows* sorted = nullptr, bool round8 = false);
hipError_t apply_small(hipStream_t s, int p, int K, int ldk, int L, int ldw, const double* d_m, const double* d_D,
                       const double* d_Vrows, const double* d_xA , const double* d_resp,
                       double* d_t, double* d_Wp, double* d_YA);
hipError_t scatter_samples(hipStream_t s, int p, int L, const long long* d_loc, const double* d_YA, float* d_Y,
                           long long ystride, bool round8 = false);

int ghist_max_cols();
size_t ghist_workspace_elems(GridSpec gs, int nrows_local);
hipError_t gram_hist(hipStream_t s, const float* d_lum, GridSpec gs, int p, int row0, int nrows_local,
                     const double* d_er, const double* d_ecT, const double* d_Ep, const double* d_c, double* d_ws,
                     double* d_Gk, LaunchObserver* obs = nullptr, const SortedRows* sorted = nullptr);

hipError_t bgr2lab8(hipStream_t s, const unsigned char* d_bgr, long long n, const double* d_lut, unsigned char* d_lab,
                    float* d_L);
hipError_t lab2bgr8(hipStream_t s, const unsigned char* d_lab, const float* d_L, const float* d_a, const float* d_b,
                    long long n, const double* d_lut, unsigned char* d_bgr);
hipError_t channel8(hipStream_t s, const unsigned char* d_img, long long n, int ch, float* d_out);
hipError_t plane_to_u8(hipStream_t s, const float* d_y, long long n, unsigned char* d_out);
hipError_t channel8_plane(hipStream_t s, const unsigned char* d_u8, long long n, float* d_out);
int bilateral8_max_radius();
hipError_t bilateral8(hipStream_t s, const float* d_src, int H, int W, int radius, const float* d_space_w,
                      const float* d_colour_w, float* d_dst);

hipError_t col_range(hipStream_t s, const float* d_X, long long M, int ld, int ncols, float* d_out, int nblocks);

hipError_t apply_expand(hipStream_t s, const float* d_V, long long M, int ld, const double* d_g,
                        int L, float* d_Y, long long ystride);

hipError_t scatter_rows(hipStream_t s, const float* d_src, const long long* d_idx, int n, int ld,
                        float* d_X, long long M);

struct ExactPlane {
    const float* lum;
    int H, W;
    const double* d_es;
    int es_len;
    const double* d_el;
    double* d_part;
};
void exact_tables(int H, int W, double hx, double hy, std::vector<double>* es, std::vector<double>* el);
size_t exact_part_elems(long long N);
hipError_t affinity_product64(hipStream_t s, const ExactPlane& pl, const double* d_X, int ldx, int ncols, double* d_Y, int ldy);
hipError_t exact_start(hipStream_t s, double* d_X, long long N, int ld, int col0, int ncols, unsigned seed);
hipError_t exact_scale2(hipStream_t s, const double* d_X, int ldx, long long N, int b, const double* d_c, const double* d_r,
                        double* d_Z);
hipError_t exact_combine(hipStream_t s, const double* d_Y, long long N, int b, const double* d_c, const double* d_r, double* d_A,
                         int lda);
hipError_t exact_recip(hipStream_t s, double* d_v, long long N, double eps);
hipError_t exact_axpby(hipStream_t s, const double* d_S, int lds, double alpha, const double* d_B, int ldb, double beta,
                       double* d_D, int ldd, long long N, int n, int pad);
int exact_col_blocks(long long N);
hipError_t exact_colnorm2(hipStream_t s, const double* d_A, int lda, const double* d_B, int ldb, const double* d_theta,
                          long long N, int n, double* d_part);
hipError_t exact_colmaxabs(hipStream_t s, const double* d_A, int lda, long long N, int n, double* d_pv);
hipError_t exact_scale_cols(hipStream_t s, double* d_A, int lda, long long N, int n, const double* d_s);

}
```

nonlocal-image-edit_amd/csrc/ortho.h:

```cpp
#pragma once
#include "devsolve.h"

namespace nlep {

constexpr double kCholMaxInvTrace = 1e9;

struct KaDevice {
    DevBuf<double> Ka;
    DevChol ch;
};

struct Nystrom {
    int r = 0, ldr = 0;
    bool chol = false;
    std::shared_ptr<KaDevice> dev;
    std::vector<double> VA;
    std::vector<double> lam;
    std::vector<double> B;
    std::vector<double> Ka;
};

struct Ortho {
    int q = 0, K = 0, r_wa = 0, r_q = 0;
    bool chol_wa = false;
    std::vector<double> Sq, Cproj, VArows, Wa;
};

struct OrthoSS {
    int q = 0, K = 0, r_wa = 0, r_q = 0;
    bool chol_wa = false;
    std::vector<double> Sq, D, Vrows;
    int p = 0, r = 0;
    std::vector<double> cA, rA, Kr, P, Wa, S, St, A2;
};

Ortho orthogonalize_host(const Nystrom& ny, int p, const std::vector<double>& u_c, const std::vector<double>& u_r,
                         std::vector<double> G, int n_eig, bool device_f32 = true, int topk_solver = 0);
void ortho_ss_prepare(OrthoSS& o, const Nystrom& ny, int p, const std::vector<double>& sA_c, const std::vector<double>& sA_r,
                      bool literal_q = false);
void ortho_ss_finish(OrthoSS& o, std::vector<double> Gk, int n_eig, int topk_solver = 0);
void ortho_ss_device(nle_ctx* c, OrthoSS& o, const Nystrom& ny, int p, const std::vector<double>& sA_c,
                     const std::vector<double>& sA_r, double* d_Gk, int n_eig, const std::function<void()>& enqueue_gram,
                     const std::function<void()>& reduce_gram, double* host_ms, double* host_overlapped_ms, Trace& tr);

}
```

nonlocal-image-edit_amd/csrc/ortho.hip:

```cpp
#include "ortho.h"

using namespace nlep;

namespace {

template <typename F>
void par_cols(int n, long long work_per_col, F&& body) {
    const long long work = work_per_col * n;
    const int nt = (int)std::min<long long>(std::min<long long>(16, work / 40000000 + 1), n);
    if (nt <= 1) {
        body(0, n);
        return;
    }
    nleh::run_parts(nt, nt, [&](int t) { body((int)((long long)n * t / nt), (int)((long long)n * (t + 1) / nt)); });
}
void mm(const double* A, const double* B, double* C, int m, int k, int n) {
    par_cols(n, (long long)m * k, [&](int j0, int j1) { nleh::gemm_nn_cols(A, B, C, m, k, n, j0, j1); });
}
void mm_nt(const double* A, const double* B, double* C, int m, int k, int n) {
    par_cols(n, (long long)m * k, [&](int j0, int j1) { nleh::gemm_nt_cols(A, B, C, m, k, n, j0, j1); });
}
void mm_tn(const double* A, const double* B, double* C, int m, int k, int n) {
    par_cols(n, (long long)m * k, [&](int j0, int j1) { nleh::gemm_tn_cols(A, B, C, m, k, n, j0, j1); });
}
// ... 491 lines not shown
        DevBuf<double> d_c2(p - q);
        HIP_OK(hipMemcpyAsync(d_c2.p, c2.data(), (p - q) * sizeof(double), hipMemcpyHostToDevice, st));
        HIP_OK(nlek::gemm64s(st, p, p, p - q, dv.Kr.p + (size_t)q * p, 1, p, dv.Kr.p + (size_t)q * p, p, 1, d_Gk, 1, p, nullptr,
                             d_c2.p, nullptr, d_Gk, 1, p));
        HIP_OK(hipStreamSynchronize(st));
    }
    if (r < p) {
        HIP_OK(nlek::gemm64s(st, p, p, p, dv.P.p, 1, p, d_Gk, 1, p, d_T.p, 1, p));
        HIP_OK(nlek::gemm64s(st, p, p, p, d_T.p, 1, p, dv.P.p, 1, p, d_Gk, 1, p));
    }
    HIP_OK(nlek::gemm64s(st, m, q, q, w.d_F.p, q, 1, d_Gk, 1, p, d_T1.p, 1, m, nullptr, dv.rA.p));
    if (!w.chol_form()) {
        HIP_OK(nlek::gemm64s(st, m, m, q, d_T1.p, 1, m, w.d_F.p, 1, q, d_Qm, 1, m, nullptr, dv.rA.p));
        return;
    }
    DevBuf<double> d_A2(qq);
    HIP_OK(nlek::gemm64s(st, q, q, q, w.d_L.p, q, 1, w.d_L.p, 1, q, d_A2.p, 1, q));
    if (w.form == WaRoot::kDeflated) {
        DevBuf<double> d_neg(w.nd);
        HIP_OK(nlek::fill64(st, d_neg.p, w.nd, -1.0));
        HIP_OK(nlek::gemm64s(st, q, q, w.nd, w.d_G.p, 1, q, w.d_G.p, q, 1, d_A2.p, 1, q, nullptr, d_neg.p, nullptr, d_A2.p, 1, q));
    }
    HIP_OK(nlek::gemm64s(st, m, m, q, d_T1.p, 1, m, w.d_F.p, 1, q, d_Qm, 1, m, nullptr, dv.rA.p, nullptr, d_A2.p, 1, q));
}

struct QtEig {
    bool on_device = false;
    std::vector<double> Vq, Sq, sv;
    DevSymEig es;
    DevBuf<double> d_Vq, d_l2q;
};

void top_eigenpairs_Qt(nle_ctx* c, OrthoSS& o, const WaRoot& w, const double* d_Qm, int n_eig, QtEig& t, double* host_ms,
                       Trace& tr) {
    hipStream_t st = c->stream;
    const int m = w.m;
    const size_t mm_ = (size_t)m * m;
    int rq = 0;
    double h0 = 0.0;
    t.on_device = c->topk_solver == 0 && use_dev_solver(m) && !std::getenv("NLE_HOST_Q");
    if (t.on_device) {
        const double* d_add = nullptr;
        if (!w.chol_form()) {
            t.d_l2q.alloc(m);
            HIP_OK(hipMemcpyAsync(t.d_l2q.p, w.l2_kept.data(), m * sizeof(double), hipMemcpyHostToDevice, st));
            d_add = t.d_l2q.p;
        }
        t.on_device = t.es.reduce(c, m, d_Qm, d_add);
        if (c->world > 1) t.on_device = ranks_where(c, !t.on_device) == 0;
    }
    if (t.on_device) {
        tr.mark("ss: Q, its tridiagonal form and eigenvalues (device)");
        h0 = now_ms();
        t.Sq = t.es.D;
        while (rq < m && t.Sq[rq] >= NLE_EPS) ++rq;
        const int Kd = std::min(n_eig, rq);
        if (Kd > 0) {
            t.d_Vq.alloc((size_t)m * Kd);
            t.es.vectors(c, 0, Kd, t.d_Vq.p);
        }
    } else {
        std::vector<double> Qm(mm_);
        HIP_OK(hipMemcpyAsync(Qm.data(), d_Qm, mm_ * sizeof(double), hipMemcpyDeviceToHost, st));
        HIP_OK(hipStreamSynchronize(st));
        tr.mark("ss: Q on the device + download");
        h0 = now_ms();
        if (!w.chol_form())
            for (int k = 0; k < m; ++k) Qm[(size_t)k * m + k] += w.l2_kept[k];
        top_eigenpairs(Qm, m, n_eig, c->topk_solver, &t.Vq, &t.Sq, &rq);
    }
    const int K = std::min(n_eig, rq);
    if (K <= 0) throw Fail{NLE_ERR_NUMERIC, "Q has no eigenvalue >= 1e-10"};
    o.K = K;
    o.r_q = rq;
    o.Sq.assign(t.Sq.begin(), t.Sq.begin() + K);
    t.sv.resize(K);
    for (int k = 0; k < K; ++k) t.sv[k] = std::sqrt(recip0(t.Sq[k]));
    *host_ms += now_ms() - h0;
    tr.mark(t.on_device ? "ss: eigenvectors of Q (inverse iteration on the host, back-transformation enqueued)" : "ss: eig(Q) (host)");
}

void D_and_Vrows(hipStream_t st, OrthoSS& o, const SsDevice& dv, const WaRoot& w, QtEig& t, const double* d_Wa, Trace& tr) {
    const int p = o.p, r = o.r, q = o.q, m = w.m, K = o.K;
    DevBuf<double> d_sv(K), d_T2((size_t)q * K), d_D((size_t)p * K), d_Vr((size_t)p * K);
    if (!t.on_device) {
        t.d_Vq.alloc((size_t)m * K);
        HIP_OK(hipMemcpyAsync(t.d_Vq.p, t.Vq.data(), (size_t)m * K * sizeof(double), hipMemcpyHostToDevice, st));
    }
    HIP_OK(hipMemcpyAsync(d_sv.p, t.sv.data(), K * sizeof(double), hipMemcpyHostToDevice, st));
    HIP_OK(nlek::gemm64s(st, q, K, m, w.d_F.p, 1, q, t.d_Vq.p, 1, m, d_T2.p, 1, q, nullptr, nullptr, d_sv.p));
    if (r < p) {
        HIP_OK(nlek::gemm64s(st, p, K, q, dv.P.p, 1, p, d_T2.p, 1, q, d_D.p, 1, p, nullptr, dv.rA.p));
    } else {
        HIP_OK(hipMemcpyAsync(d_D.p, d_T2.p, (size_t)q * K * sizeof(double), hipMemcpyDeviceToDevice, st));
        HIP_OK(nlek::scale_rows64(st, d_D.p, p, K, dv.rA.p));
    }
    HIP_OK(nlek::gemm64s(st, q, K, q, d_Wa, 1, q, d_T2.p, 1, q, d_Vr.p, 1, p));
    if (q < p)
        HIP_OK(nlek::gemm64s(st, p - q, K, p, dv.Kr.p + q, 1, p, d_D.p, 1, p, d_Vr.p + q, 1, p, dv.cA.p + q));
    o.D.resize((size_t)p * K);
    o.Vrows.resize((size_t)p * K);
    HIP_OK(hipMemcpyAsync(o.D.data(), d_D.p, o.D.size() * sizeof(double), hipMemcpyDeviceToHost, st));
    HIP_OK(hipMemcpyAsync(o.Vrows.data(), d_Vr.p, o.Vrows.size() * sizeof(double), hipMemcpyDeviceToHost, st));
    HIP_OK(hipStreamSynchronize(st));
    tr.mark("ss: D, Vrows on the device");
}

}

void ortho_ss_device(nle_ctx* c, OrthoSS& o, const Nystrom& ny, int p, const std::vector<double>& sA_c,
                     const std::vector<double>& sA_r, double* d_Gk, int n_eig, const std::function<void()>& enqueue_gram,
                     const std::function<void()>& reduce_gram, double* host_ms, double* host_overlapped_ms, Trace& tr) {
    const int q = ny.r;
    hipStream_t st = c->stream;
    SsDevice dv;
    scalings_Kr_P(st, o, ny, p, sA_c, sA_r, dv);
    const double h0 = now_ms();
    const bool dev_wa = use_dev_solver(q) && !std::getenv("NLE_HOST_WA");
    const bool force_eig = std::getenv("NLE_FORCE_EIG") != nullptr;
    if (!(dev_wa && ny.dev)) build_Wa(o);
    DevBuf<double> d_Wa((size_t)q * q);
    WaRoot w;
    WaDeviceWork ws;
    if (dev_wa)
        wa_root_device(c, o, ny, dv, d_Wa.p, force_eig, enqueue_gram, ws, w, tr);
    else
        enqueue_gram();
    if (!w.on_device) wa_root_host(o, !dev_wa, force_eig, w, tr);
    o.r_wa = w.r_wa;
    o.chol_wa = w.form == WaRoot::kCholesky;
    *host_overlapped_ms += now_ms() - h0;
    tr.mark(w.on_device ? "ss: Wa root (device, second stream, beside the Gram kernels)" : "ss: Wa root (host, under the Gram kernels)");
    w.m = w.chol_form() ? q : std::max(w.r_wa, 0);
    if (w.m <= 0) throw Fail{NLE_ERR_NUMERIC, "Wa has no eigenvalue >= 1e-10"};
    DevBuf<double> d_Qm((size_t)w.m * w.m);
    if (!dev_wa) HIP_OK(hipMemcpyAsync(d_Wa.p, o.Wa.data(), (size_t)q * q * sizeof(double), hipMemcpyHostToDevice, st));
    if (!w.on_device) upload_host_root(st, q, w);
    form_Qt(st, o, dv, w, d_Gk, reduce_gram, d_Qm.p);
    QtEig t;
    top_eigenpairs_Qt(c, o, w, d_Qm.p, n_eig, t, host_ms, tr);
    D_and_Vrows(st, o, dv, w, t, d_Wa.p, tr);
}

}
```

nonlocal-image-edit_amd/csrc/pipeline.hip:

```cpp
#include "ortho.h"
#include "samples.h"

using nlek::GridSpec;
using namespace nlep;

namespace {
GridSpec checked_grid(int H, int W, int nRow, int nCol) {
    check_image_size(H, W);
    if (nRow > H || nCol > W)
        throw Fail{NLE_ERR_INVALID, "Number of samples per row and col must be <= that of image."};
    GridSpec gs;
    if (!make_grid(H, W, nRow, nCol, &gs)) throw Fail{NLE_ERR_INVALID, "invalid sample counts"};
    return gs;
}



Nystrom solve_Ka(nle_ctx* c, const std::vector<double>& Ka, int p, bool allow_chol) {
    Nystrom n;
    if (allow_chol && std::getenv("NLE_FORCE_EIG") == nullptr) {
        if (c && use_dev_solver(p) && !std::getenv("NLE_HOST_KA")) {
            const size_t pp = (size_t)p * p;
            auto kd = std::make_shared<KaDevice>();
            kd->Ka.alloc(pp);
// ... 343 lines not shown
        HIP_OK(hipMemsetAsync(d_X1.p, 0, n2 * p * sizeof(double), c->stream));
        HIP_OK(nlek::transpose64(c->stream, p, ny.dev->ch.Linv.p, d_X1.p, p, 2 * p));
        HIP_OK(hipMemcpyAsync(d_X2.p, ny.dev->ch.Linv.p, pp * sizeof(double), hipMemcpyDeviceToDevice, c->stream));
        HIP_OK(hipMemcpyAsync(d_X2.p + pp, ny.dev->Ka.p, pp * sizeof(double), hipMemcpyDeviceToDevice, c->stream));
        HIP_OK(nlek::fill64(c->stream, d_lam.p, p, 1.0));
    } else {
        const size_t n2 = (size_t)2 * p;
        std::vector<double> X1(n2 * r, 0.0), X2(n2 * r);
        for (int k = 0; k < r; ++k)
            for (int a = 0; a < p; ++a) {
                const double b = ny.B[(size_t)k * p + a];
                const double va = ny.chol ? ny.Ka[(size_t)k * p + a] : ny.VA[(size_t)k * p + a];
                X1[(size_t)k * n2 + a] = b;
                if (!ny.chol) X1[(size_t)k * n2 + p + a] = va;
                X2[(size_t)a * r + k] = b;
                X2[(size_t)(p + a) * r + k] = va;
            }
        d_X1.alloc(X1.size());
        d_X2.alloc(X2.size());
        d_lam.alloc(r);
        HIP_OK(hipMemcpyAsync(d_X1.p, X1.data(), X1.size() * sizeof(double), hipMemcpyHostToDevice, c->stream));
        HIP_OK(hipMemcpyAsync(d_X2.p, X2.data(), X2.size() * sizeof(double), hipMemcpyHostToDevice, c->stream));
        HIP_OK(hipMemcpyAsync(d_lam.p, ny.lam.data(), r * sizeof(double), hipMemcpyHostToDevice, c->stream));
        HIP_OK(hipStreamSynchronize(c->stream));
    }
}

struct SampleSinkhorn {
    nle_ctx* c;
    int p, T, zld;
    DevBuf<double> d_w, d_sAh, d_X1, d_X2, d_lam, d_uv;
    std::vector<double> sA_c, sA_r;

    SampleSinkhorn(nle_ctx* c_, int p_, int zld_, int T_)
        : c(c_), p(p_), T(T_), zld(zld_), d_w(zld_), d_sAh((size_t)2 * T_ * p_), d_uv((size_t)3 * p_) {
        HIP_OK(hipMemsetAsync(d_w.p, 0, zld * sizeof(double), c->stream));
    }

    Nystrom run(const std::function<Nystrom()>& solve, const std::function<void(int, bool)>& pass_pixels, double* d_z,
                int zrows) {
        pass_pixels(nlek::ROWPASS_COLSUM, false);
        Nystrom ny = solve();
        build_update_operands(c, ny, p, d_X1, d_X2, d_lam);
        auto update = [&](int n, int mode) {
            all_reduce(c, d_z, (size_t)zrows * zld);
            PROFILED(c, NLE_K_SMALL,
                     nlek::sink_update(c->stream, mode, p, ny.r, ny.chol, d_X1.p, d_X2.p, d_lam.p, d_z, zrows, zld,
                                       n > 0 ? d_sAh.p + (size_t)(n - 1) * p : nullptr, NLE_EPS, d_uv.p, d_uv.p + 2 * p,
                                       d_sAh.p + (size_t)n * p, d_w.p));
        };
        update(0, nlek::ROWPASS_COLSUM);
        for (int n = 1; n < 2 * T; ++n) {
            pass_pixels(nlek::ROWPASS_RECIP, n == 2 * T - 1);
            update(n, nlek::ROWPASS_RECIP);
        }
        sA_c.resize(p);
        sA_r.resize(p);
        HIP_OK(hipMemcpyAsync(sA_c.data(), d_sAh.p + (size_t)(2 * T - 2) * p, p * sizeof(double), hipMemcpyDeviceToHost,
                              c->stream));
        HIP_OK(hipMemcpyAsync(sA_r.data(), d_sAh.p + (size_t)(2 * T - 1) * p, p * sizeof(double), hipMemcpyDeviceToHost,
                              c->stream));
        return ny;
    }
};

void train_sample_space(nle_ctx* c, nle_filter* f, const float* d_lum, const SampleSet& ss,
                        const std::function<Nystrom()>& solve, double hx, double hy, int T, int n_eig, long long pix0,
                        long long M, StageMs* ms) {
    const int p = ss.p;
    const int P64 = nlek::sink_pass_ld(p);
    const float nsw = nsw_of(hx), npw = nsw_of(hy);
    Trace tr;
    Timer tm_s(c->stream), tm_g(c->stream), tm_p(c->stream);
    tm_s.start();
    DevBuf<float4> d_samples = upload_samples(c, ss, P64);
    constexpr int kZS = 8;
    const int npart = nlek::sink_pass_rows(std::max<long long>(M, 1));
    DevBuf<double> d_z((size_t)kZS * P64), d_partial, d_cbuf((size_t)std::max<long long>(M, 1));
    const bool hist = ss.quantised && c->mode != NLE_MODE_PHI_FREE_EXP && ss.gs.nSelCols <= nlek::ghist_max_cols() &&
                      ss.gs.nSelRows <= 32 && M > 0;
    if (!hist && p > nlek::sink_pass_max_p()) throw Fail{NLE_ERR_INVALID, "Phi-free path: too many samples for the generic kernels"};
    const int nrows_local = (int)(M / ss.gs.W), row0 = (int)(pix0 / ss.gs.W);
    DevBuf<double> d_er, d_ecT, d_Ep, d_hws;
    if (hist) {
        d_er.alloc((size_t)nrows_local * ss.gs.nSelRows);
        d_ecT.alloc((size_t)ss.gs.nSelCols * ss.gs.W);
        d_Ep.alloc((size_t)256 * p);
        d_hws.alloc(nlek::hist_tiled_workspace_elems(ss.gs, nrows_local));
        PROFILED(c, NLE_K_SMALL, nlek::hist_tables(c->stream, ss.gs, d_samples.p, p, hx, hy, row0, nrows_local, d_er.p,
                                                   d_ecT.p, d_Ep.p));
    } else {
        d_partial.alloc((size_t)npart * P64);
    }
    SampleSinkhorn sk(c, p, P64, T);
    const bool sorted = hist && ss.gs.W <= nlek::sorted_max_width() && std::getenv("NLE_NO_SORTED_ROWS") == nullptr;
    DevBuf<unsigned short> d_scol, d_first;
    DevBuf<uint2> d_desc;
    DevBuf<double> d_E, d_E2;
    nlek::SortedRows sr{};
    if (sorted) {
        d_scol.alloc(nlek::sorted_scol_elems(ss.gs.W, nrows_local));
        d_first.alloc((size_t)nrows_local * 258);
        d_desc.alloc((size_t)nrows_local * nlek::kSortedThreads);
        d_E.alloc((size_t)ss.gs.W + 1);
        PROFILED(c, NLE_K_SMALL, nlek::dist_table(c->stream, ss.gs.W, hx, d_E.p));
        PROFILED(c, NLE_K_SMALL, nlek::sort_rows(c->stream, d_lum, ss.gs, row0, nrows_local, d_scol.p, d_desc.p, d_first.p));
        HIP_OK(hipMemsetAsync(d_cbuf.p, 0, d_cbuf.n * sizeof(double), c->stream));
        sr = nlek::SortedRows{d_scol.p, d_desc.p, d_first.p, d_E.p, false, 0.0};
        sr.rec = nlek::sorted_recurrence(ss.gs, hx, &sr.kappa);
        sr.mom = nlek::sorted_moments_ok(ss.gs, hx);
        if (std::getenv("NLE_ALL_LEVEL_TILES") == nullptr) {
            int t0 = 0, t1 = 16;
            while (t0 < 15 && !((ss.level_tiles >> t0) & 1u)) ++t0;
            while (t1 > t0 + 1 && !((ss.level_tiles >> (t1 - 1)) & 1u)) --t1;
            sr.lev_t0 = t0;
            sr.lev_nt = t1 - t0;
        }
        if (nlek::sorted_gsum_ok(ss.gs, hx)) {
            d_E2.alloc((size_t)ss.gs.W + 1);
            PROFILED(c, NLE_K_SMALL, nlek::dist_table(c->stream, ss.gs.W, hx / std::sqrt(2.0), d_E2.p));
            sr.E2 = d_E2.p;
            sr.hx = hx;
        }
    }
    const nlek::SortedRows* srp = sorted ? &sr : nullptr;
    tr.mark("ss: alloc+upload");
    auto pass_pixels = [&](int mode, bool last) {
        double* ybuf = last ? d_cbuf.p : nullptr;
        if (hist) {
            static const int kmap[4] = {NLE_K_SINK_TABLES, NLE_K_SINKHORN_PASS, NLE_K_REDUCE, NLE_K_REDUCE};
            ProfObserver obs(c, kmap);
            HIP_OK(nlek::sink_hist_tiled(c->stream, mode, d_lum, ss.gs, p, P64, row0, nrows_local, d_er.p, d_ecT.p,
                                         d_Ep.p, sk.d_w.p, NLE_EPS, ybuf, d_hws.p, d_z.p, &obs, nullptr, nullptr, srp));
        } else if (M > 0) {
            PROFILED(c, NLE_K_SINKHORN_PASS, nlek::sink_pass(c->stream, mode, d_lum, ss.gs, d_samples.p, p, sk.d_w.p, nsw,
                                                             npw, pix0, M, NLE_EPS, ybuf, d_partial.p));
            PROFILED(c, NLE_K_REDUCE, nlek::reduce_partials(c->stream, d_partial.p, npart, P64, d_z.p, kZS));
        } else {
            HIP_OK(hipMemsetAsync(d_z.p, 0, (size_t)kZS * P64 * sizeof(double), c->stream));
        }
    };
    const Nystrom ny = sk.run(solve, pass_pixels, d_z.p, hist ? 1 : kZS);
    f->r = ny.r;
    f->chol_ka = ny.chol ? 1 : 0;
    f->formulation = hist ? NLE_MODE_PHI_FREE : NLE_MODE_PHI_FREE_EXP;
    tm_s.stop();
    tr.mark("ss: passes enqueued");
    HIP_OK(hipStreamSynchronize(c->stream));
    tr.mark("ss: sinkhorn sync");

    tm_g.start();
    const int ntiles = nlek::gram64_num_tiles(p);
    const size_t g_elems = hist ? (size_t)p * p : (size_t)ntiles * 256;
    DevBuf<double> d_gpart, d_tiles(g_elems);
    auto enqueue_gram = [&] {
        if (M <= 0) {
            HIP_OK(hipMemsetAsync(d_tiles.p, 0, g_elems * sizeof(double), c->stream));
        } else if (hist) {
            d_gpart.alloc(nlek::ghist_workspace_elems(ss.gs, nrows_local));
            static const int gmap[4] = {NLE_K_GRAM_ROWS, NLE_K_SMALL, NLE_K_GRAM_GEMM, NLE_K_SMALL};
            ProfObserver obs(c, gmap);
            HIP_OK(nlek::gram_hist(c->stream, d_lum, ss.gs, p, row0, nrows_local, d_er.p, d_ecT.p, d_Ep.p, d_cbuf.p,
                                   d_gpart.p, d_tiles.p, &obs, srp));
        } else {
            d_gpart.alloc(std::max<size_t>(nlek::gram64_partial_elems(M, p), 1));
            PROFILED(c, NLE_K_GRAM, nlek::gram64(c->stream, d_lum, ss.gs, d_samples.p, p, nsw, npw, pix0, M, d_cbuf.p,
                                                 d_gpart.p, d_tiles.p));
        }
    };
    OrthoSS o;
    if (hist && c->topk_solver == 0) {
        ortho_ss_device(c, o, ny, p, sk.sA_c, sk.sA_r, d_tiles.p, n_eig, enqueue_gram,
                        [&] { all_reduce(c, d_tiles.p, g_elems); }, &ms->host, &ms->host_overlapped, tr);
        tm_g.stop();
    } else {
        enqueue_gram();
        double h0 = now_ms();
        ortho_ss_prepare(o, ny, p, sk.sA_c, sk.sA_r, c->topk_solver != 0);
        const double h_overlapped = now_ms() - h0;
        tr.mark("ss: ortho prepare (host)");
        all_reduce(c, d_tiles.p, g_elems);
        std::vector<double> tiles(g_elems);
        HIP_OK(hipMemcpyAsync(tiles.data(), d_tiles.p, tiles.size() * sizeof(double), hipMemcpyDeviceToHost, c->stream));
        tm_g.stop();
        HIP_OK(hipStreamSynchronize(c->stream));
        tr.mark("ss: gram sync");
        h0 = now_ms();
        ortho_ss_finish(o, hist ? std::move(tiles) : unpack_tiles(tiles, nlek::gram64_ld(p), p, 16), n_eig, c->topk_solver);
        ms->host += now_ms() - h0;
        tr.mark("ss: ortho finish (host)");
        ms->host_overlapped += h_overlapped;
    }
    adopt_ortho(f, o);

    tm_p.start();
    if (o.K > 128) throw Fail{NLE_ERR_INVALID, "Phi-free path supports at most 128 eigenvectors"};
    const int ldd = nlek::project64_ld(o.K);
    std::vector<double> Dp((size_t)p * ldd, 0.0);
    for (int k = 0; k < o.K; ++k)
        for (int a = 0; a < p; ++a) Dp[(size_t)a * ldd + k] = o.D[(size_t)k * p + a];
    DevBuf<double> d_D(Dp.size());
    HIP_OK(hipMemcpyAsync(d_D.p, Dp.data(), Dp.size() * sizeof(double), hipMemcpyHostToDevice, c->stream));
    if (hist) {
        auto own = [&](auto& buf) {
            using T = std::remove_pointer_t<decltype(buf.p)>;
            const size_t bytes = buf.n * sizeof(T);
            T* ptr = buf.take();
            f->owned.emplace_back(ptr, bytes);
            return ptr;
        };
        std::vector<double> Vr((size_t)p * ldd, 0.0);
        for (int k = 0; k < o.K; ++k)
            for (int a = 0; a < p; ++a) Vr[(size_t)a * ldd + k] = o.Vrows[(size_t)k * p + a];
        DevBuf<double> d_Vr(Vr.size());
        DevBuf<long long> d_spix(p), d_sloc(p);
        DevBuf<float> d_slab((size_t)M);
        std::vector<long long> sloc(p);
        for (int a = 0; a < p; ++a) {
            const long long loc = ss.pix[a] - pix0;
            sloc[a] = (loc >= 0 && loc < M) ? loc : -1;
        }
        HIP_OK(hipMemcpyAsync(d_Vr.p, Vr.data(), Vr.size() * sizeof(double), hipMemcpyHostToDevice, c->stream));
        HIP_OK(hipMemcpyAsync(d_spix.p, ss.pix.data(), p * sizeof(long long), hipMemcpyHostToDevice, c->stream));
        HIP_OK(hipMemcpyAsync(d_sloc.p, sloc.data(), p * sizeof(long long), hipMemcpyHostToDevice, c->stream));
        HIP_OK(hipMemcpyAsync(d_slab.p, d_lum + pix0, (size_t)M * sizeof(float), hipMemcpyDeviceToDevice, c->stream));
        HIP_OK(hipStreamSynchronize(c->stream));
        f->lazy = true;
        f->gs = ss.gs;
        f->nsw = nsw;
        f->npw = npw;
        f->ldd = ldd;
        f->P64 = P64;
        f->d_lum = own(d_slab);
        f->d_c = own(d_cbuf);
        f->d_er = own(d_er);
        f->d_ecT = own(d_ecT);
        f->d_Ep = own(d_Ep);
        f->d_D = own(d_D);
        f->d_Vrows = own(d_Vr);
        f->d_samples = own(d_samples);
        f->d_sample_pix = own(d_spix);
        f->d_sample_loc = own(d_sloc);
        if (sorted) {
            f->has_sorted = true;
            f->sorted = nlek::SortedRows{own(d_scol), own(d_desc), own(d_first), own(d_E), sr.rec, sr.kappa};
            f->sorted.lev_t0 = sr.lev_t0;
            f->sorted.lev_nt = sr.lev_nt;
            f->sorted.mom = sr.mom;
        }
        f->h_Vrows = o.Vrows;
        f->h_sample_pix = ss.pix;
        tm_p.stop();
        ms->take(tm_s, tm_g, tm_p);
        return;
    }
    DevBuf<float> d_V((size_t)std::max<long long>(M, 1) * f->ldv);
    PROFILED(c, NLE_K_PROJECT, nlek::project64(c->stream, d_lum, ss.gs, d_samples.p, p, nsw, npw, pix0, M, d_D.p, o.K,
                                               d_cbuf.p, d_V.p, f->ldv));
    tr.mark("ss: project enqueued");
    scatter_sample_rows(c, ss.pix, p, o.Vrows, o.K, f->ldv, pix0, M, d_V.p);
    tm_p.stop();
    HIP_OK(hipStreamSynchronize(c->stream));
    tr.mark("ss: project sync");
    f->v_bytes = d_V.n * sizeof(float);
    f->d_V = d_V.take();
    ms->take(tm_s, tm_g, tm_p);
}

void train_stream64(nle_ctx* c, nle_filter* f, const float* d_lum, const SampleSet& ss, const std::function<Nystrom()>& solve,
                    double hx, double hy, int T, int n_eig, long long pix0, long long M, StageMs* ms) {
    const int p = ss.p, ld = ld4(p);
    hipStream_t st = c->stream;
    Trace tr;
    Timer tm_s(st), tm_g(st), tm_p(st);
    tm_s.start();
    size_t budget_mb = 2048;
    if (const char* e = std::getenv("NLE_STREAM64_CHUNK_MB")) budget_mb = (size_t)std::max(1, std::atoi(e));
    const long long rows_fit = (long long)((budget_mb << 20) / ((size_t)ld * sizeof(double)));
    const long long CH = std::max<long long>(256, std::min<long long>(std::max<long long>(M, 1), rows_fit));
    const AffinityRows64 kab(c, d_lum, ss, hx, hy, true);
    DevBuf<double> d_K((size_t)CH * ld), d_partial((size_t)nlek::kRowpassMaxBlocks * ld), d_zc(ld), d_z(ld), d_ones(ld),
        d_cbuf((size_t)std::max<long long>(M, 1));
    SampleSinkhorn sk(c, p, ld, T);
    HIP_OK(nlek::fill64(st, d_ones.p, ld, 1.0));
    tr.mark("s64: alloc+upload");
    auto chunk_rows = [&](long long i0) { return std::min<long long>(CH, M - i0); };
    auto gen = [&](long long i0, long long mc) { PROFILED(c, NLE_K_AFFINITY, kab.rows(pix0 + i0, mc, d_K.p, true)); };
    auto pass_pixels = [&](int mode, bool last) {
        HIP_OK(hipMemsetAsync(d_z.p, 0, ld * sizeof(double), st));
        for (long long i0 = 0; i0 < M; i0 += CH) {
            const long long mc = chunk_rows(i0);
            gen(i0, mc);
            int nb = 0;
            PROFILED(c, NLE_K_SINKHORN_PASS, nlek::rowpass64(st, mode, d_K.p, mc, ld, ld, sk.d_w.p, d_ones.p, nullptr, NLE_EPS, d_partial.p, &nb));
            PROFILED(c, NLE_K_REDUCE, nlek::reduce_partials(st, d_partial.p, nb, ld, d_zc.p));
            HIP_OK(nlek::add64(st, d_z.p, d_zc.p, ld));
            if (last) PROFILED(c, NLE_K_SMALL, nlek::row_scalings64(st, d_K.p, mc, ld, p, sk.d_w.p, NLE_EPS, d_cbuf.p + i0));
        }
    };
    const Nystrom ny = sk.run(solve, pass_pixels, d_z.p, 1);
    f->r = ny.r;
    f->chol_ka = ny.chol ? 1 : 0;
    f->formulation = NLE_MODE_STREAMED_F64;
    tm_s.stop();
    HIP_OK(hipStreamSynchronize(st));
    tr.mark("s64: sinkhorn");
    tm_g.start();
    const size_t pp = (size_t)p * p;
    DevBuf<double> d_G(pp), d_Gc(pp), d_gpart(std::max<size_t>(nlek::gram64d_partial_elems(CH, p), 1));
// ... 1207 lines not shown
```

nonlocal-image-edit_amd/csrc/pipeline_internal.h:

```cpp
#pragma once
#include <hip/hip_runtime.h>
#include <dlfcn.h>
#include <rccl/rccl.h>

#include <algorithm>
#include <atomic>
#include <mutex>
#include <functional>
#include <chrono>
#include <cmath>
#include <cstdio>
#include <cstdlib>
#include <cstring>
#include <map>
#include <memory>
#include <set>
#include <string>
#include <thread>
#include <type_traits>
#include <vector>

#include "../../include/nle.h"
#include "eigen_sym.h"
#include "kernels.h"
// ... 59 lines not shown
    double ms[6] = {0, 0, 0, 0, 0, 0};
    int formulation = 0, r_wa = 0, r_q = 0, chol_ka = 0, chol_wa = 0;
    bool lazy = false;
    nlek::GridSpec gs{};
    float nsw = 0.f, npw = 0.f;
    int ldd = 0, P64 = 0;
    float* d_plane = nullptr;
    size_t plane_bytes = 0;
    float* d_lum = nullptr;
    double *d_c = nullptr, *d_er = nullptr, *d_ecT = nullptr, *d_Ep = nullptr, *d_D = nullptr, *d_Vrows = nullptr;
    float4* d_samples = nullptr;
    long long *d_sample_pix = nullptr, *d_sample_loc = nullptr;
    bool has_sorted = false;
    nlek::SortedRows sorted{};
    std::vector<std::pair<void*, size_t>> owned;
    std::vector<double> h_Vrows;
    std::vector<long long> h_sample_pix;
};


namespace nlep {

struct Fail {
    int code;
    std::string msg;
};

#define HIP_OK(expr)                                                                              \
    do {                                                                                          \
        hipError_t e_ = (expr);                                                                   \
        if (e_ != hipSuccess)                                                                     \
            throw Fail{NLE_ERR_HIP, std::string(#expr) + ": " + hipGetErrorString(e_)};           \
    } while (0)

inline thread_local nle_ctx* g_cur = nullptr;
struct CurCtx {
    nle_ctx* prev;
    explicit CurCtx(nle_ctx* c) : prev(g_cur) { g_cur = c; }
    ~CurCtx() { g_cur = prev; }
};

inline void* arena_alloc(nle_ctx* c, size_t bytes) {
    if (c) {
        auto it = c->arena_free.lower_bound(bytes);
        if (it != c->arena_free.end() && it->first <= bytes + bytes / 4 + 4096) {
            void* p = it->second;
            c->arena_free.erase(it);
            return p;
        }
    }
    void* p = nullptr;
    hipError_t e = hipMalloc(&p, bytes);
    if (e != hipSuccess && c && !c->arena_free.empty()) {
        (void)hipStreamSynchronize(c->stream);
        for (auto& kv : c->arena_free) (void)hipFree(kv.second);
        c->arena_free.clear();
        c->arena_bytes = 0;
        e = hipMalloc(&p, bytes);
    }
    if (e != hipSuccess) throw Fail{NLE_ERR_HIP, std::string("hipMalloc: ") + hipGetErrorString(e)};
    if (c) c->arena_bytes += bytes;
    return p;
}

inline void arena_release(nle_ctx* c, void* p, size_t bytes) {
    if (!p) return;
    if (c) {
        c->arena_free.emplace(bytes, p);
    } else {
        (void)hipFree(p);
    }
}

template <typename T>
struct DevBuf {
    T* p = nullptr;
    size_t n = 0;
    nle_ctx* owner = nullptr;
    DevBuf() = default;
    explicit DevBuf(size_t count) { alloc(count); }
    DevBuf(const DevBuf&) = delete;
    DevBuf& operator=(const DevBuf&) = delete;
    DevBuf(DevBuf&& o) noexcept : p(o.p), n(o.n), owner(o.owner) { o.take(); }
    void alloc(size_t count) {
        release();
        if (count) {
            owner = g_cur;
            p = static_cast<T*>(arena_alloc(owner, count * sizeof(T)));
        }
        n = count;
    }
    void release() {
        if (p) arena_release(owner, p, n * sizeof(T));
        p = nullptr;
        n = 0;
    }
    T* take() {
        T* q = p;
        p = nullptr;
        n = 0;
        return q;
    }
    ~DevBuf() { release(); }
};

struct Timer {
    hipEvent_t a = nullptr, b = nullptr;
    hipStream_t s;
    explicit Timer(hipStream_t st) : s(st) {
        HIP_OK(hipEventCreate(&a));
        HIP_OK(hipEventCreate(&b));
    }
    ~Timer() {
        if (a) (void)hipEventDestroy(a);
        if (b) (void)hipEventDestroy(b);
    }
    void start() { HIP_OK(hipEventRecord(a, s)); }
    void stop() { HIP_OK(hipEventRecord(b, s)); }
    double ms() {
        HIP_OK(hipEventSynchronize(b));
        float t = 0.f;
        HIP_OK(hipEventElapsedTime(&t, a, b));
        return t;
    }
};

inline int ld4(int n) { return (n + 3) & ~3; }

constexpr double kLog2e = 1.4426950408889634074;
inline float nsw_of(double h) { return (float)(-kLog2e / (h * h)); }

inline hipEvent_t prof_event(nle_ctx* c) {
    if (!c->prof_pool.empty()) {
        hipEvent_t e = c->prof_pool.back();
        c->prof_pool.pop_back();
        return e;
    }
    hipEvent_t e = nullptr;
    HIP_OK(hipEventCreate(&e));
    return e;
}

struct Prof {
    nle_ctx* c;
    int kid;
    hipEvent_t a = nullptr, b = nullptr;
    Prof(nle_ctx* c_, int kid_) : c(c_), kid(kid_) {
        if (!c->profiling) return;
        if (!c->profile_all && (kid == NLE_K_SMALL || kid == NLE_K_REDUCE || kid == NLE_K_SINK_TABLES)) return;
        a = prof_event(c);
        b = prof_event(c);
        HIP_OK(hipEventRecord(a, c->stream));
    }
    void end() {
        if (!a) return;
        HIP_OK(hipEventRecord(b, c->stream));
        c->prof_pending.push_back({kid, a, b});
        a = nullptr;
    }
};

#define PROFILED(ctx_, kid_, expr)  \
    do {                            \
        Prof pf_((ctx_), (kid_));   \
        HIP_OK(expr);               \
        pf_.end();                  \
// ... 191 lines not shown
```

nonlocal-image-edit_amd/csrc/sorted.hip:

```cpp
#include "kernels.h"

#include <algorithm>
#include <cmath>
#include <cstdlib>

#define NLE_PIXEL_FENCE() __builtin_amdgcn_sched_barrier(0)

namespace nlek {

namespace {
constexpr int kLevels = 256;
constexpr int kT = kSortedThreads;
constexpr int kSortThreads = 256;

__device__ __forceinline__ double recip0_d(double s, double eps) {
    double r = __builtin_amdgcn_rcp(s);
    r = fma(fma(-s, r, 1.0), r, r);
    r = fma(fma(-s, r, 1.0), r, r);
    return (fabs(s) >= eps) ? r : 0.0;
}

using lds_cdouble_ptr = const __attribute__((address_space(3))) double*;
__device__ __forceinline__ unsigned lds_addr(const void* p) {
    return (unsigned)(unsigned long long)(const __attribute__((address_space(3))) char*)p;
// ... 437 lines not shown
                    const unsigned c8[PB] = {idx[b].x & 0xffffu, idx[b].x >> 16, idx[b].y & 0xffffu, idx[b].y >> 16};
                    pixels(c8, 4 * b);
                    NLE_PIXEL_FENCE();
                } else if constexpr (PB == 2) {
                    const unsigned c8a[PB] = {idx[b].x & 0xffffu, idx[b].x >> 16}, c8b[PB] = {idx[b].y & 0xffffu, idx[b].y >> 16};
                    pixels(c8a, 4 * b);
                    NLE_PIXEL_FENCE();
                    if (4 * b + 2 < wlen) {
                        pixels(c8b, 4 * b + 2);
                        NLE_PIXEL_FENCE();
                    }
                } else {
                    const unsigned cs4[4] = {idx[b].x & 0xffffu, idx[b].x >> 16, idx[b].y & 0xffffu, idx[b].y >> 16};
#pragma unroll
                    for (int k = 0; k < 4; ++k) {
                        if (4 * b + k < wlen) {
                            const unsigned c8one[PB] = {cs4[k]};
                            pixels(c8one, 4 * b + k);
                            NLE_PIXEL_FENCE();
                        }
                    }
                }
            }
        } else {
#pragma unroll
        for (int b = 0; b < kMaxBlocks; ++b) {
            if (4 * b >= wlen) break;
            pixel(idx[b].x & 0xffffu, 4 * b < len);
            NLE_PIXEL_FENCE();
            if (4 * b + 1 < wlen) {
                pixel(idx[b].x >> 16, 4 * b + 1 < len);
                NLE_PIXEL_FENCE();
            }
            if (4 * b + 2 < wlen) {
                pixel(idx[b].y & 0xffffu, 4 * b + 2 < len);
                NLE_PIXEL_FENCE();
            }
            if (4 * b + 3 < wlen) {
                pixel(idx[b].y >> 16, 4 * b + 3 < len);
                NLE_PIXEL_FENCE();
            }
        }
        }
        if constexpr (MOM) {
#pragma unroll
            for (int b = 2; b < NC; ++b) acc[b] *= sCk[b];
        }
        __builtin_amdgcn_s_setprio(3);
        if (has_next && recip) {
            if constexpr (PRE) {
#pragma unroll
                for (int b = 0; b < NC; ++b) gv[b] = gvn[b];
            } else {
#pragma unroll
                for (int b = 0; b < NC; ++b) gv[b] = g[(size_t)nrow * n + b * kLevels + dsc_level(dsc_n)];
            }
        }
        double* hrow = hout + (size_t)lrow * n;
#pragma unroll
        for (int s0 = 0; s0 < NC; s0 += SL) {
            double v[SL];
#pragma unroll
            for (int i = 0; i < SL; ++i) v[i] = (s0 + i < NC) ? acc[s0 + i] : 0.0;
#pragma unroll
            for (int i = 0; i < SL; ++i) sP[tid * PS + i] = v[i];
            __syncthreads();
            if (s0 == 0) {
                asm volatile("" ::"v"(sf_n), "v"(dsc_nn.x), "v"(dsc_nn.y));
#pragma unroll
                for (int b = 0; b < kMaxBlocks; ++b) asm volatile("" ::"v"(idx_n[b].x), "v"(idx_n[b].y));
#pragma unroll
                for (int b = 0; b < NC; ++b) asm volatile("" ::"v"(gv[b]));
                if (has_next && tid < 258) sfirst[(par ^ 1) * 260 + tid] = sf_n;
            }
            const int ns = (NC - s0 < SL) ? NC - s0 : SL;
            const int nlev = lev_nt * 16, xlo = lev_t0 * 16;
            const float inv_nlev = 1.0f / (float)nlev;
            for (int i = tid; i < ns * nlev; i += kT) {
                const int bb = (int)(((float)i + 0.5f) * inv_nlev);
                const int xx = xlo + (i - bb * nlev);
                const int f0 = sfc[xx], f1 = sfc[xx + 1];
                double sum = 0.0;
                for (int t = f0; t < f1; ++t) sum += sP[t * PS + bb];
                hrow[(size_t)(s0 + bb) * kLevels + xx] = sum;
            }
            __syncthreads();
        }
        __builtin_amdgcn_s_setprio(0);
        if (!has_next) break;
        lrow = nrow;
        nrow = nnrow;
        dsc = dsc_n;
        dsc_n = dsc_nn;
#pragma unroll
        for (int b = 0; b < kMaxBlocks; ++b) idx[b] = idx_n[b];
    }
}

static int sorted_grid(int nrows) {
    int ncu = 256;
    int dev = 0;
    if (hipGetDevice(&dev) == hipSuccess) (void)hipDeviceGetAttribute(&ncu, hipDeviceAttributeMultiprocessorCount, dev);
    int mult = 2;
    if (const char* e = std::getenv("NLE_SORTED_WGS_PER_CU")) mult = std::max(1, std::atoi(e));
    return std::max(1, std::min(nrows, mult * ncu));
}

bool sorted_recurrence(GridSpec gs, double hx, double* kappa) {
    const double cs = gs.colStep, umax = std::max<double>(gs.colOff, gs.W - 1 - gs.colOff), nC = gs.nSelCols;
    const double span = umax + nC * cs;
    const double m_e = span * span / (hx * hx);
    const double m_rho = (2.0 * cs * umax + (2.0 * nC + 1.0) * cs * cs) / (hx * hx);
    *kappa = std::exp(-2.0 * cs * cs / (hx * hx));
    const bool off = std::getenv("NLE_SORTED_TABLE") != nullptr;
    return !off && gs.nSelCols > 12 && m_e < 500.0 && m_rho < 500.0;
}

bool sorted_moments_ok(GridSpec gs, double hx) {
    if (std::getenv("NLE_SORTED_TABLE") != nullptr || std::getenv("NLE_SORTED_NO_MOMENTS") != nullptr) return false;
    const double cs = gs.colStep, umax = std::max<double>(gs.colOff, gs.W - 1 - gs.colOff), nC = gs.nSelCols;
    const double span = umax + nC * cs;
    return span * span / (hx * hx) < 500.0;
}

hipError_t sorted_pass(hipStream_t s, int mode, GridSpec gs, int row0, int nrows_local, const unsigned short* d_scol,
                       const uint2* d_desc, const unsigned short* d_first, const double* d_E, const double* d_g, double eps,
                       double* d_ybuf, double* d_h, const double* d_cvec, const float* d_xvec, bool rec, double kappa,
                       int lev_t0, int lev_nt, bool mom) {
    const int nC = gs.nSelCols;
    if (nC < 1 || nC > 36 || gs.W > sorted_max_width() || lev_t0 < 0 || lev_nt < 1 || lev_t0 + lev_nt > kLevels / 16)
        return hipErrorInvalidValue;
    if (nrows_local <= 0) return hipSuccess;
    const size_t shm = sorted_lds_bytes(gs.W, (nC < 11 ? nC : 11) | 1);
    const int grid = sorted_grid(nrows_local);
#define NLE_SP1(NCV, CFV)                                                                                                 \
    {                                                                                                                     \
        if (shm > 48 * 1024) {                                                                                            \
            hipError_t ea = hipFuncSetAttribute(reinterpret_cast<const void*>(k_sorted_pass<NCV, CFV>),                   \
                                                hipFuncAttributeMaxDynamicSharedMemorySize, (int)shm);                    \
            if (ea != hipSuccess) return ea;                                                                              \
        }                                                                                                                 \
        hipLaunchKernelGGL((k_sorted_pass<NCV, CFV>), dim3((unsigned)grid), dim3(kT), shm, s, mode, d_scol, d_desc,        \
                           d_first, gs, row0, nrows_local, d_E, d_g, eps, d_ybuf, d_h, d_cvec, d_xvec, kappa, lev_t0,     \
                           lev_nt);                                                                                       \
    }
#define NLE_SP(NCV)                                                                                                       \
    case NCV:                                                                                                             \
        if constexpr ((NCV) > 1) {                                                                                        \
            if (mom) {                                                                                                    \
                NLE_SP1(NCV, 2)                                                                                           \
                break;                                                                                                    \
            }                                                                                                             \
        }                                                                                                                 \
        if constexpr ((NCV) > 12) {                                                                                       \
            if (rec) NLE_SP1(NCV, 1) else NLE_SP1(NCV, 0)                                                                 \
        } else {                                                                                                          \
            if (rec) return hipErrorInvalidValue;                                                                         \
            NLE_SP1(NCV, 0)                                                                                               \
        }                                                                                                                 \
        break;
    switch (nC) {
        NLE_SP(1) NLE_SP(2) NLE_SP(3) NLE_SP(4) NLE_SP(5) NLE_SP(6) NLE_SP(7) NLE_SP(8) NLE_SP(9) NLE_SP(10) NLE_SP(11)
        NLE_SP(12) NLE_SP(13) NLE_SP(14) NLE_SP(15) NLE_SP(16) NLE_SP(17) NLE_SP(18) NLE_SP(19) NLE_SP(20)
        NLE_SP(21) NLE_SP(22) NLE_SP(23) NLE_SP(24) NLE_SP(25) NLE_SP(26) NLE_SP(27) NLE_SP(28) NLE_SP(29)
        NLE_SP(30) NLE_SP(31) NLE_SP(32) NLE_SP(33) NLE_SP(34) NLE_SP(35) NLE_SP(36)
        default: return hipErrorInvalidValue;
    }
// ... 456 lines not shown
```

Measured before the change: 3311 MP/s.

## Keep D and Vrows on device, unroll gemm64s k-loop, add test entry points

Packs D and Vrows into a row-major padded layout on the device and hands those buffers to the filter setup, replacing the host-side transpose and re-upload. The sample index and slab uploads move earlier so they can overlap, the gemm64s inner loop gets deeper k-unrolling with a templated dk path, and some histogram and gram stores become relaxed atomic stores. It also exposes gemm64s and sink_update through the C ABI and Python for testing. The device-to-host copy of D and Vrows is kept so the host copies stay filled, so the PCIe traffic is only partly removed.

```diff
diff --git a/include/nle.h b/include/nle.h
--- a/include/nle.h
+++ b/include/nle.h
@@ -104,6 +104,12 @@
 int nle_ts_gemm64(nle_ctx* ctx, const double* d_A, long long M, int lda, int kd, const double* h_B, int nc, double* d_C);
 int nle_sinkhorn_scalings64(nle_ctx* ctx, const double* d_phi, long long M, int ld, int r, const double* h_eigvals,
                             int max_iter, double* h_u_c, double* h_u_r);
+int nle_gemm64s(nle_ctx* ctx, int m, int n, int k, const double* d_A, long long rsA, long long csA, const double* d_B,
+                long long rsB, long long csB, double* d_C, long long rsC, long long csC, const double* d_dl,
+                const double* d_dk, const double* d_dr, const double* d_add, long long rsD, long long csD);
+int nle_sink_update(nle_ctx* ctx, int mode, int p, int r, int chol, const double* d_X1, const double* d_X2,
+                    const double* d_lam, const double* d_zpart, int nparts, int ldp, const double* d_sA_cur, double* d_z,
+                    double* d_u, double* d_sA_next, double* d_w);
 int nle_gram64(nle_ctx* ctx, const double* d_phi, long long M, int ld, int r, const double* h_u, double* h_G);
 int nle_row_scalings64(nle_ctx* ctx, const double* d_phi, long long M, int ld, int r, const double* h_u, double* d_out);
 int nle_affinity_product64(nle_ctx* ctx, const float* d_lum, int H, int W, double hx, double hy, const double* d_X, int ld,
diff --git a/nonlocal-image-edit_amd/__init__.py b/nonlocal-image-edit_amd/__init__.py
--- a/nonlocal-image-edit_amd/__init__.py
+++ b/nonlocal-image-edit_amd/__init__.py
@@ -496,6 +496,49 @@
                                    C.c_void_p(Cc.data_ptr())), self._h)
         return Cc
 
+    def gemm64s(self, A, B, dl=None, dk=None, dr=None, add=None, out=None):
+        torch = _torch()
+        for t_, nd in ((A, 2), (B, 2), (add, 2), (out, 2), (dl, 1), (dk, 1), (dr, 1)):
+            if t_ is not None and (t_.dtype != torch.float64 or t_.ndim != nd or not t_.is_cuda):
+                raise NLEError(NLE_ERR_INVALID, "gemm64s: need float64 device tensors")
+        (m, k), n = A.shape, B.shape[1]
+        if B.shape[0] != k or any(v is not None and (v.numel() != sz or not v.is_contiguous())
+                                  for v, sz in ((dl, m), (dk, k), (dr, n))):
+            raise NLEError(NLE_ERR_INVALID, "gemm64s: operand shapes do not match")
+        if out is None:
+            out = torch.empty((m, n), dtype=torch.float64, device=A.device)
+        if tuple(out.shape) != (m, n) or (add is not None and tuple(add.shape) != (m, n)):
+            raise NLEError(NLE_ERR_INVALID, "gemm64s: add and out must be m x n")
+        self._sync_in()
+        ptr = lambda t_: C.c_void_p(t_.data_ptr()) if t_ is not None else None
+        _check(lib().nle_gemm64s(self._h, m, n, k, ptr(A), A.stride(0), A.stride(1), ptr(B), B.stride(0), B.stride(1),
+                                 ptr(out), out.stride(0), out.stride(1), ptr(dl), ptr(dk), ptr(dr), ptr(add),
+                                 add.stride(0) if add is not None else 0, add.stride(1) if add is not None else 0), self._h)
+        return out
+
+    def sink_update(self, mode, X1, X2, lam, zpart, p, sA_cur=None, chol=False):
+        torch = _torch()
+        dev = zpart.device
+        as_dev = lambda a: torch.as_tensor(np.ascontiguousarray(a, dtype=np.float64), device=dev)
+        X1d, X2d, lamd = as_dev(X1), as_dev(X2), as_dev(lam)
+        r = X2d.shape[1]
+        if X1d.shape != (r, 2 * p) or X2d.shape != (2 * p, r) or lamd.numel() != r or zpart.dtype != torch.float64 \
+                or zpart.ndim != 2 or not zpart.is_contiguous() or zpart.shape[1] < p:
+            raise NLEError(NLE_ERR_INVALID, "sink_update: operand shapes do not match")
+        nparts, ldp = zpart.shape
+        sAd = as_dev(sA_cur) if sA_cur is not None else None
+        z = torch.full((ldp,), float("nan"), dtype=torch.float64, device=dev)
+        w = torch.full((ldp,), float("nan"), dtype=torch.float64, device=dev)
+        u = torch.empty(r, dtype=torch.float64, device=dev)
+        sA = torch.empty(p, dtype=torch.float64, device=dev)
+        self._sync_in()
+        _check(lib().nle_sink_update(self._h, int(mode), p, r, 1 if chol else 0, C.c_void_p(X1d.data_ptr()),
+                                     C.c_void_p(X2d.data_ptr()), C.c_void_p(lamd.data_ptr()), C.c_void_p(zpart.data_ptr()),
+                                     nparts, ldp, C.c_void_p(sAd.data_ptr()) if sAd is not None else None,
+                                     C.c_void_p(z.data_ptr()), C.c_void_p(u.data_ptr()), C.c_void_p(sA.data_ptr()),
+                                     C.c_void_p(w.data_ptr())), self._h)
+        return z.cpu().numpy(), u.cpu().numpy(), sA.cpu().numpy(), w.cpu().numpy()
+
     def sinkhorn_scalings64(self, phi, r, eigvals, max_iter=10):
         M, ldp = self._mat64(phi, r, "sinkhorn_scalings64")
         ev = np.ascontiguousarray(eigvals, dtype=np.float64)
diff --git a/nonlocal-image-edit_amd/_abi.py b/nonlocal-image-edit_amd/_abi.py
--- a/nonlocal-image-edit_amd/_abi.py
+++ b/nonlocal-image-edit_amd/_abi.py
@@ -83,6 +83,8 @@
     "nle_compute_kernel64": (C.c_int, [_P, _P, C.c_int, C.c_int, C.c_int, C.c_int, C.c_double, C.c_double, _P, _P]),
     "nle_ts_gemm64": (C.c_int, [_P, _P, C.c_longlong, C.c_int, C.c_int, _P, C.c_int, _P]),
     "nle_sinkhorn_scalings64": (C.c_int, [_P, _P, C.c_longlong, C.c_int, C.c_int, _P, C.c_int, _P, _P]),
+    "nle_gemm64s": (C.c_int, [_P, C.c_int, C.c_int, C.c_int, _P, C.c_longlong, C.c_longlong, _P, C.c_longlong, C.c_longlong, _P, C.c_longlong, C.c_longlong, _P, _P, _P, _P, C.c_longlong, C.c_longlong]),
+    "nle_sink_update": (C.c_int, [_P, C.c_int, C.c_int, C.c_int, C.c_int, _P, _P, _P, _P, C.c_int, C.c_int, _P, _P, _P, _P, _P]),
     "nle_gram64": (C.c_int, [_P, _P, C.c_longlong, C.c_int, C.c_int, _P, _P]),
     "nle_row_scalings64": (C.c_int, [_P, _P, C.c_longlong, C.c_int, C.c_int, _P, _P]),
     "nle_affinity_product64": (C.c_int, [_P, _P, C.c_int, C.c_int, C.c_double, C.c_double, _P, C.c_int, C.c_int, _P]),
diff --git a/nonlocal-image-edit_amd/csrc/abi_ctx.hip b/nonlocal-image-edit_amd/csrc/abi_ctx.hip
--- a/nonlocal-image-edit_amd/csrc/abi_ctx.hip
+++ b/nonlocal-image-edit_amd/csrc/abi_ctx.hip
@@ -492,4 +492,34 @@
     });
 }
 
-}
+int nle_gemm64s(nle_ctx* ctx, int m, int n, int k, const double* d_A, long long rsA, long long csA, const double* d_B,
+                long long rsB, long long csB, double* d_C, long long rsC, long long csC, const double* d_dl,
+                const double* d_dk, const double* d_dr, const double* d_add, long long rsD, long long csD) {
+    if (!ctx || !d_A || !d_B || !d_C || m < 1 || n < 1 || k < 1) return NLE_ERR_INVALID;
+    return guard(ctx, [&] {
+        HIP_OK(hipSetDevice(ctx->device));
+        HIP_OK(nlek::gemm64s(ctx->stream, m, n, k, d_A, rsA, csA, d_B, rsB, csB, d_C, rsC, csC, d_dl, d_dk, d_dr, d_add, rsD,
+                             csD));
+        HIP_OK(hipStreamSynchronize(ctx->stream));
+    });
+}
+
+int nle_sink_update(nle_ctx* ctx, int mode, int p, int r, int chol, const double* d_X1, const double* d_X2,
+                    const double* d_lam, const double* d_zpart, int nparts, int ldp, const double* d_sA_cur, double* d_z,
+                    double* d_u, double* d_sA_next, double* d_w) {
+    if (!ctx || !d_X1 || !d_X2 || !d_lam || !d_zpart || !d_z || !d_u || !d_sA_next || !d_w || p < 1 || r < 1 || nparts < 1 ||
+        ldp < p || (mode != nlek::ROWPASS_COLSUM && mode != nlek::ROWPASS_RECIP) || (mode == nlek::ROWPASS_RECIP && !d_sA_cur) ||
+        (chol && r != p))
+        return NLE_ERR_INVALID;
+    return guard(ctx, [&] {
+        HIP_OK(hipSetDevice(ctx->device));
+        DevBuf<double> d_v((size_t)2 * p);
+        HIP_OK(hipMemsetAsync(d_w, 0, (size_t)ldp * sizeof(double), ctx->stream));
+        HIP_OK(nlek::z_reduce(ctx->stream, d_zpart, nparts, p, ldp, d_z));
+        HIP_OK(nlek::sink_update(ctx->stream, mode, p, r, chol != 0, d_X1, d_X2, d_lam, d_z, 1, ldp, d_sA_cur, NLE_EPS, d_v.p,
+                                 d_u, d_sA_next, d_w));
+        HIP_OK(hipStreamSynchronize(ctx->stream));
+    });
+}
+
+}
diff --git a/nonlocal-image-edit_amd/csrc/fused.hip b/nonlocal-image-edit_amd/csrc/fused.hip
--- a/nonlocal-image-edit_amd/csrc/fused.hip
+++ b/nonlocal-image-edit_amd/csrc/fused.hip
@@ -817,7 +817,7 @@
 #pragma unroll
             for (int e = 0; e < 4; ++e) {
                 const int ro = t * 16 + kq + 4 * e;
-                if (ro < nrows) g[(size_t)ro * n + col] = acc[e];
+                if (ro < nrows) __hip_atomic_store(&g[(size_t)ro * n + col], acc[e], __ATOMIC_RELAXED, __HIP_MEMORY_SCOPE_AGENT);
             }
         }
     }
@@ -1086,6 +1086,11 @@
         for (int k = 0; k < 32; ++k) t += sm[k][c];
         z[col] = t;
     }
+}
+
+hipError_t z_reduce(hipStream_t s, const double* d_zpart, int nparts, int p, int ldp, double* d_z) {
+    hipLaunchKernelGGL(k_z_reduce, dim3((unsigned)((ldp + 7) / 8)), dim3(256), 0, s, d_zpart, nparts, p, ldp, d_z);
+    return hipGetLastError();
 }
 
 int hist_tiled_max_rows_samples() { return 32; }
@@ -1172,8 +1177,7 @@
         hipLaunchKernelGGL(k_hist_hh, dim3((unsigned)((nC * lev_nt + 3) / 4), (unsigned)nslabs), dim3(256), shm_hh, s, nC, nR,
                            nrows_local, slab_rows, lev_t0, lev_nt, d_er, d_h, d_Ep, p, ldp, d_HH);
     }
-    hipLaunchKernelGGL(k_z_reduce, dim3((unsigned)((ldp + 7) / 8)), dim3(256), 0, s, d_HH, nslabs * lev_nt, p, ldp, d_z);
-    return hipGetLastError();
+    return z_reduce(s, d_HH, nslabs * lev_nt, p, ldp, d_z);
 }
 
 int apply_layers_per_launch(GridSpec gs) {
diff --git a/nonlocal-image-edit_amd/csrc/generic64.hip b/nonlocal-image-edit_amd/csrc/generic64.hip
--- a/nonlocal-image-edit_amd/csrc/generic64.hip
+++ b/nonlocal-image-edit_amd/csrc/generic64.hip
@@ -193,6 +193,41 @@
     return hipGetLastError();
 }
 
+constexpr int kGsSpan = 7;
+template <bool HAS_DK>
+__device__ __forceinline__ f64x4 gemm64s_tile(const int kk, const int kq, const bool aok, const bool bok,
+                                              const double* __restrict__ ap, const long long csA,
+                                              const double* __restrict__ bp, const long long rsB,
+                                              const double* __restrict__ dk) {
+    f64x4 acc = f64x4{0.0, 0.0, 0.0, 0.0};
+    for (int k0 = 0; k0 < kk; k0 += 16 * kGsSpan) {
+        double a[kGsSpan][4], b[kGsSpan][4], d[HAS_DK ? kGsSpan : 1][4];
+#pragma unroll
+        for (int s = 0; s < kGsSpan; ++s) {
+#pragma unroll
+            for (int u = 0; u < 4; ++u) {
+                const int k = k0 + 16 * s + 4 * u + kq;
+                const bool kok = k < kk;
+                a[s][u] = (aok && kok) ? ap[(long long)k * csA] : 0.0;
+                b[s][u] = (bok && kok) ? bp[(long long)k * rsB] : 0.0;
+                if constexpr (HAS_DK) d[s][u] = (aok && kok) ? dk[k] : 0.0;
+            }
+        }
+#pragma unroll
+        for (int s = 0; s < kGsSpan; ++s) {
+            if (k0 + 16 * s < kk) {
+#pragma unroll
+                for (int u = 0; u < 4; ++u) {
+                    double av = a[s][u];
+                    if constexpr (HAS_DK) av = (aok && k0 + 16 * s + 4 * u + kq < kk) ? av * d[s][u] : 0.0;
+                    acc = __builtin_amdgcn_mfma_f64_16x16x4f64(av, b[s][u], acc, 0, 0, 0);
+                }
+            }
+        }
+    }
+    return acc;
+}
+
 __global__ __launch_bounds__(256) void k_gemm64s(int m, int n, int kk, const double* __restrict__ A, long long rsA,
                                                  long long csA, const double* __restrict__ B, long long rsB, long long csB,
                                                  double* __restrict__ C, long long rsC, long long csC,
@@ -208,19 +243,8 @@
     const bool aok = ai < m, bok = bj < n;
     const double* ap = A + (long long)ai * rsA;
     const double* bp = B + (long long)bj * csB;
-    f64x4 acc = f64x4{0.0, 0.0, 0.0, 0.0};
-    for (int k0 = 0; k0 < kk; k0 += 16) {
-        double a[4], b[4];
-#pragma unroll
-        for (int u = 0; u < 4; ++u) {
-            const int k = k0 + 4 * u + kq;
-            const bool kok = k < kk;
-            a[u] = (aok && kok) ? ap[(long long)k * csA] * (dk ? dk[k] : 1.0) : 0.0;
-            b[u] = (bok && kok) ? bp[(long long)k * rsB] : 0.0;
-        }
-#pragma unroll
-        for (int u = 0; u < 4; ++u) acc = __builtin_amdgcn_mfma_f64_16x16x4f64(a[u], b[u], acc, 0, 0, 0);
-    }
+    const f64x4 acc = dk ? gemm64s_tile<true>(kk, kq, aok, bok, ap, csA, bp, rsB, dk)
+                         : gemm64s_tile<false>(kk, kq, aok, bok, ap, csA, bp, rsB, dk);
     if (bok) {
         const double sr = dr ? dr[bj] : 1.0;
 #pragma unroll
@@ -450,13 +474,25 @@
     return hipGetLastError();
 }
 
-__global__ void k_scale_rows64(double* __restrict__ X, int m, int n, const double* __restrict__ dl) {
+__global__ void k_pack_rows64(const double* __restrict__ A, const double* __restrict__ dl, const double* __restrict__ B,
+                              int m, int n, int ld, double* __restrict__ outA, double* __restrict__ outB) {
     const long long f = (long long)blockIdx.x * blockDim.x + threadIdx.x;
-    if (f < (long long)m * n) X[f] *= dl[f % m];
-}
-hipError_t scale_rows64(hipStream_t s, double* d_X, int m, int n, const double* d_dl) {
-    if (m <= 0 || n <= 0) return hipSuccess;
-    hipLaunchKernelGGL(k_scale_rows64, dim3((unsigned)(((long long)m * n + 255) / 256)), dim3(256), 0, s, d_X, m, n, d_dl);
+    if (f >= (long long)m * ld) return;
+    const int i = (int)(f / ld), j = (int)(f - (long long)i * ld);
+    double a = 0.0, b = 0.0;
+    if (j < n) {
+        a = A[(size_t)j * m + i];
+        if (dl) a *= dl[i];
+        b = B[(size_t)j * m + i];
+    }
+    outA[f] = a;
+    outB[f] = b;
+}
+hipError_t pack_rows64(hipStream_t s, const double* d_A, const double* d_dl, const double* d_B, int m, int n, int ld,
+                       double* d_outA, double* d_outB) {
+    if (m <= 0 || ld <= 0) return hipSuccess;
+    hipLaunchKernelGGL(k_pack_rows64, dim3((unsigned)(((long long)m * ld + 255) / 256)), dim3(256), 0, s, d_A, d_dl, d_B, m, n,
+                       ld, d_outA, d_outB);
     return hipGetLastError();
 }
 
diff --git a/nonlocal-image-edit_amd/csrc/kernels.h b/nonlocal-image-edit_amd/csrc/kernels.h
--- a/nonlocal-image-edit_amd/csrc/kernels.h
+++ b/nonlocal-image-edit_amd/csrc/kernels.h
@@ -151,7 +151,8 @@
                           long long ystride);
 hipError_t scatter_rows64(hipStream_t s, const double* d_src, const long long* d_idx, int n, int ld, double* d_X, long long M);
 hipError_t to_f32(hipStream_t s, const double* d_X, long long n, float* d_out);
-hipError_t scale_rows64(hipStream_t s, double* d_X, int m, int n, const double* d_dl);
+hipError_t pack_rows64(hipStream_t s, const double* d_A, const double* d_dl, const double* d_B, int m, int n, int ld,
+                       double* d_outA, double* d_outB);
 
 int tridiag_max_n();
 hipError_t tridiag(hipStream_t s, int n, const double* d_Q, const double* d_diag_add, double* d_V, double* d_d, double* d_e,
@@ -212,6 +213,7 @@
                             double kappa);
 
 size_t hist_tiled_workspace_elems(GridSpec gs, int nrows_local);
+hipError_t z_reduce(hipStream_t s, const double* d_zpart, int nparts, int p, int ldp, double* d_z);
 hipError_t sink_hist_tiled(hipStream_t s, int mode, const float* d_lum, GridSpec gs, int p, int ldp, int row0,
                            int nrows_local, const double* d_er, const double* d_ecT, const double* d_Ep,
                            const double* d_w, double eps, double* d_ybuf, double* d_ws, double* d_z,
diff --git a/nonlocal-image-edit_amd/csrc/ortho.h b/nonlocal-image-edit_amd/csrc/ortho.h
--- a/nonlocal-image-edit_amd/csrc/ortho.h
+++ b/nonlocal-image-edit_amd/csrc/ortho.h
@@ -30,6 +30,8 @@
     int q = 0, K = 0, r_wa = 0, r_q = 0;
     bool chol_wa = false;
     std::vector<double> Sq, D, Vrows;
+    DevBuf<double> d_D, d_Vrows;
+    int ldd = 0;
     int p = 0, r = 0;
     std::vector<double> cA, rA, Kr, P, Wa, S, St, A2;
 };
diff --git a/nonlocal-image-edit_amd/csrc/ortho.hip b/nonlocal-image-edit_amd/csrc/ortho.hip
--- a/nonlocal-image-edit_amd/csrc/ortho.hip
+++ b/nonlocal-image-edit_amd/csrc/ortho.hip
@@ -597,7 +597,7 @@
 
 void D_and_Vrows(hipStream_t st, OrthoSS& o, const SsDevice& dv, const WaRoot& w, QtEig& t, const double* d_Wa, Trace& tr) {
     const int p = o.p, r = o.r, q = o.q, m = w.m, K = o.K;
-    DevBuf<double> d_sv(K), d_T2((size_t)q * K), d_D((size_t)p * K), d_Vr((size_t)p * K);
+    DevBuf<double> d_sv(K), d_T2((size_t)q * K), d_D, d_Vr((size_t)p * K);
     if (!t.on_device) {
         t.d_Vq.alloc((size_t)m * K);
         HIP_OK(hipMemcpyAsync(t.d_Vq.p, t.Vq.data(), (size_t)m * K * sizeof(double), hipMemcpyHostToDevice, st));
@@ -605,19 +605,28 @@
     HIP_OK(hipMemcpyAsync(d_sv.p, t.sv.data(), K * sizeof(double), hipMemcpyHostToDevice, st));
     HIP_OK(nlek::gemm64s(st, q, K, m, w.d_F.p, 1, q, t.d_Vq.p, 1, m, d_T2.p, 1, q, nullptr, nullptr, d_sv.p));
     if (r < p) {
+        d_D.alloc((size_t)p * K);
         HIP_OK(nlek::gemm64s(st, p, K, q, dv.P.p, 1, p, d_T2.p, 1, q, d_D.p, 1, p, nullptr, dv.rA.p));
-    } else {
-        HIP_OK(hipMemcpyAsync(d_D.p, d_T2.p, (size_t)q * K * sizeof(double), hipMemcpyDeviceToDevice, st));
-        HIP_OK(nlek::scale_rows64(st, d_D.p, p, K, dv.rA.p));
     }
     HIP_OK(nlek::gemm64s(st, q, K, q, d_Wa, 1, q, d_T2.p, 1, q, d_Vr.p, 1, p));
     if (q < p)
         HIP_OK(nlek::gemm64s(st, p - q, K, p, dv.Kr.p + q, 1, p, d_D.p, 1, p, d_Vr.p + q, 1, p, dv.cA.p + q));
+    const int ldd = nlek::project64_ld(K);
+    o.ldd = ldd;
+    o.d_D.alloc((size_t)p * ldd);
+    o.d_Vrows.alloc((size_t)p * ldd);
+    HIP_OK(nlek::pack_rows64(st, r < p ? d_D.p : d_T2.p, r < p ? nullptr : dv.rA.p, d_Vr.p, p, K, ldd, o.d_D.p, o.d_Vrows.p));
+    std::vector<double> Dp((size_t)p * ldd), Vp((size_t)p * ldd);
+    HIP_OK(hipMemcpyAsync(Dp.data(), o.d_D.p, Dp.size() * sizeof(double), hipMemcpyDeviceToHost, st));
+    HIP_OK(hipMemcpyAsync(Vp.data(), o.d_Vrows.p, Vp.size() * sizeof(double), hipMemcpyDeviceToHost, st));
+    HIP_OK(hipStreamSynchronize(st));
     o.D.resize((size_t)p * K);
     o.Vrows.resize((size_t)p * K);
-    HIP_OK(hipMemcpyAsync(o.D.data(), d_D.p, o.D.size() * sizeof(double), hipMemcpyDeviceToHost, st));
-    HIP_OK(hipMemcpyAsync(o.Vrows.data(), d_Vr.p, o.Vrows.size() * sizeof(double), hipMemcpyDeviceToHost, st));
-    HIP_OK(hipStreamSynchronize(st));
+    for (int a = 0; a < p; ++a)
+        for (int k = 0; k < K; ++k) {
+            o.D[(size_t)k * p + a] = Dp[(size_t)a * ldd + k];
+            o.Vrows[(size_t)k * p + a] = Vp[(size_t)a * ldd + k];
+        }
     tr.mark("ss: D, Vrows on the device");
 }
 
diff --git a/nonlocal-image-edit_amd/csrc/pipeline.hip b/nonlocal-image-edit_amd/csrc/pipeline.hip
--- a/nonlocal-image-edit_amd/csrc/pipeline.hip
+++ b/nonlocal-image-edit_amd/csrc/pipeline.hip
@@ -449,7 +449,19 @@
     if (!hist && p > nlek::sink_pass_max_p()) throw Fail{NLE_ERR_INVALID, "Phi-free path: too many samples for the generic kernels"};
     const int nrows_local = (int)(M / ss.gs.W), row0 = (int)(pix0 / ss.gs.W);
     DevBuf<double> d_er, d_ecT, d_Ep, d_hws;
+    DevBuf<long long> d_spix, d_sloc;
+    DevBuf<float> d_slab;
+    std::vector<long long> sloc;
     if (hist) {
+        d_spix.alloc(p);
+        d_sloc.alloc(p);
+        sloc.resize(p);
+        for (int a = 0; a < p; ++a) {
+            const long long loc = ss.pix[a] - pix0;
+            sloc[a] = (loc >= 0 && loc < M) ? loc : -1;
+        }
+        HIP_OK(hipMemcpyAsync(d_spix.p, ss.pix.data(), p * sizeof(long long), hipMemcpyHostToDevice, c->stream));
+        HIP_OK(hipMemcpyAsync(d_sloc.p, sloc.data(), p * sizeof(long long), hipMemcpyHostToDevice, c->stream));
         d_er.alloc((size_t)nrows_local * ss.gs.nSelRows);
         d_ecT.alloc((size_t)ss.gs.nSelCols * ss.gs.W);
         d_Ep.alloc((size_t)256 * p);
@@ -491,6 +503,10 @@
         }
     }
     const nlek::SortedRows* srp = sorted ? &sr : nullptr;
+    if (hist) {
+        d_slab.alloc((size_t)M);
+        HIP_OK(hipMemcpyAsync(d_slab.p, d_lum + pix0, (size_t)M * sizeof(float), hipMemcpyDeviceToDevice, c->stream));
+    }
     tr.mark("ss: alloc+upload");
     auto pass_pixels = [&](int mode, bool last) {
         double* ybuf = last ? d_cbuf.p : nullptr;
@@ -563,11 +579,18 @@
     tm_p.start();
     if (o.K > 128) throw Fail{NLE_ERR_INVALID, "Phi-free path supports at most 128 eigenvectors"};
     const int ldd = nlek::project64_ld(o.K);
-    std::vector<double> Dp((size_t)p * ldd, 0.0);
-    for (int k = 0; k < o.K; ++k)
-        for (int a = 0; a < p; ++a) Dp[(size_t)a * ldd + k] = o.D[(size_t)k * p + a];
-    DevBuf<double> d_D(Dp.size());
-    HIP_OK(hipMemcpyAsync(d_D.p, Dp.data(), Dp.size() * sizeof(double), hipMemcpyHostToDevice, c->stream));
+    const bool on_dev = o.d_D.p != nullptr && o.d_Vrows.p != nullptr && o.ldd == ldd;
+    std::vector<double> Dp, Vr;
+    DevBuf<double> d_D;
+    if (on_dev) {
+        d_D = std::move(o.d_D);
+    } else {
+        Dp.assign((size_t)p * ldd, 0.0);
+        for (int k = 0; k < o.K; ++k)
+            for (int a = 0; a < p; ++a) Dp[(size_t)a * ldd + k] = o.D[(size_t)k * p + a];
+        d_D.alloc(Dp.size());
+        HIP_OK(hipMemcpyAsync(d_D.p, Dp.data(), Dp.size() * sizeof(double), hipMemcpyHostToDevice, c->stream));
+    }
     if (hist) {
         auto own = [&](auto& buf) {
             using T = std::remove_pointer_t<decltype(buf.p)>;
@@ -576,22 +599,17 @@
             f->owned.emplace_back(ptr, bytes);
             return ptr;
         };
-        std::vector<double> Vr((size_t)p * ldd, 0.0);
-        for (int k = 0; k < o.K; ++k)
-            for (int a = 0; a < p; ++a) Vr[(size_t)a * ldd + k] = o.Vrows[(size_t)k * p + a];
-        DevBuf<double> d_Vr(Vr.size());
-        DevBuf<long long> d_spix(p), d_sloc(p);
-        DevBuf<float> d_slab((size_t)M);
-        std::vector<long long> sloc(p);
-        for (int a = 0; a < p; ++a) {
-            const long long loc = ss.pix[a] - pix0;
-            sloc[a] = (loc >= 0 && loc < M) ? loc : -1;
-        }
-        HIP_OK(hipMemcpyAsync(d_Vr.p, Vr.data(), Vr.size() * sizeof(double), hipMemcpyHostToDevice, c->stream));
-        HIP_OK(hipMemcpyAsync(d_spix.p, ss.pix.data(), p * sizeof(long long), hipMemcpyHostToDevice, c->stream));
-        HIP_OK(hipMemcpyAsync(d_sloc.p, sloc.data(), p * sizeof(long long), hipMemcpyHostToDevice, c->stream));
-        HIP_OK(hipMemcpyAsync(d_slab.p, d_lum + pix0, (size_t)M * sizeof(float), hipMemcpyDeviceToDevice, c->stream));
-        HIP_OK(hipStreamSynchronize(c->stream));
+        DevBuf<double> d_Vr;
+        if (on_dev) {
+            d_Vr = std::move(o.d_Vrows);
+        } else {
+            Vr.assign((size_t)p * ldd, 0.0);
+            for (int k = 0; k < o.K; ++k)
+                for (int a = 0; a < p; ++a) Vr[(size_t)a * ldd + k] = o.Vrows[(size_t)k * p + a];
+            d_Vr.alloc(Vr.size());
+            HIP_OK(hipMemcpyAsync(d_Vr.p, Vr.data(), Vr.size() * sizeof(double), hipMemcpyHostToDevice, c->stream));
+            HIP_OK(hipStreamSynchronize(c->stream));
+        }
         f->lazy = true;
         f->gs = ss.gs;
         f->nsw = nsw;
diff --git a/nonlocal-image-edit_amd/csrc/pipeline_internal.h b/nonlocal-image-edit_amd/csrc/pipeline_internal.h
--- a/nonlocal-image-edit_amd/csrc/pipeline_internal.h
+++ b/nonlocal-image-edit_amd/csrc/pipeline_internal.h
@@ -165,6 +165,16 @@
     DevBuf(const DevBuf&) = delete;
     DevBuf& operator=(const DevBuf&) = delete;
     DevBuf(DevBuf&& o) noexcept : p(o.p), n(o.n), owner(o.owner) { o.take(); }
+    DevBuf& operator=(DevBuf&& o) noexcept {
+        if (this != &o) {
+            release();
+            p = o.p;
+            n = o.n;
+            owner = o.owner;
+            o.take();
+        }
+        return *this;
+    }
     void alloc(size_t count) {
         release();
         if (count) {
diff --git a/nonlocal-image-edit_amd/csrc/sorted.hip b/nonlocal-image-edit_amd/csrc/sorted.hip
--- a/nonlocal-image-edit_amd/csrc/sorted.hip
+++ b/nonlocal-image-edit_amd/csrc/sorted.hip
@@ -543,7 +543,7 @@
                 const int f0 = sfc[xx], f1 = sfc[xx + 1];
                 double sum = 0.0;
                 for (int t = f0; t < f1; ++t) sum += sP[t * PS + bb];
-                hrow[(size_t)(s0 + bb) * kLevels + xx] = sum;
+                __hip_atomic_store(&hrow[(size_t)(s0 + bb) * kLevels + xx], sum, __ATOMIC_RELAXED, __HIP_MEMORY_SCOPE_AGENT);
             }
             __syncthreads();
         }
```

Result: no change. 3277 MP/s (median of 5 runs) (-1.0%).
